# zfwangDP/X2-GNN

Hardware: AMD Instinct MI355X
Metric: molecules/sec (fwd+bwd) on QM9 U0, batch=128, 1/2/4/8 MI355X (higher is better)
Workload: dtype fp32; 1 GPU; xgnn_poly U0 train step (config.json: L=4, D=128, H=16, sbf 7x6), S160, fwd+loss+bwd+allreduce+clip+Adam+EMA; per_gpu_batch=128, global_batch=128, line_nodes_per_gpu=21058, triplets_per_gpu=194060, parallelism=dp1, hip_graph=True

## Files before the change

### x2-gnn_amd/csrc/chain.hip

```cpp
#include <math.h>

#include <type_traits>

#include "common.hpp"

namespace x2g {
namespace {

typedef float f4 __attribute__((ext_vector_type(4)));

constexpr int kCD = 128;
constexpr int kCWaves = 8;
constexpr int kCThreads = kCWaves * 64;

struct ChainFwdArgs {
  const float* x;
  const float* res;
  float* in_t;
  int64_t tf;
  int64_t R;
  int n;
  x2g_chain_stage st[X2G_CHAIN_MAX_STAGES];
};

struct ChainBwdArgs {
  const float* dy;
  const float* dy_add;
  float* dx;
  float* dres;
  float* dz_t;
  const float* ln_y;
  float2* ln_gstats;
  int64_t tf;
  int64_t R;
  int n;
  x2g_chain_bwd_stage st[X2G_CHAIN_MAX_STAGES];
};

__device__ __forceinline__ f4 zero4() { return f4{0.f, 0.f, 0.f, 0.f}; }

__device__ __forceinline__ float sigmoid_fast(float z) {
  return __builtin_amdgcn_rcpf(1.0f + __builtin_amdgcn_exp2f(-1.4426950408889634f * z));
}
__device__ __forceinline__ float silu_fast(float z) { return z * sigmoid_fast(z); }
__device__ __forceinline__ float silu_grad_fast(float z) {
  const float s = sigmoid_fast(z);
  return s * (1.0f + z * (1.0f - s));
}

constexpr int kV2RB = 6;

__device__ __forceinline__ int ipos(int r, int c) { return r * 32 + (c ^ (r & 15)); }

typedef __amdgpu_buffer_rsrc_t rsrc_t;

__device__ __forceinline__ rsrc_t rsrc(const float* p) {
  return __builtin_amdgcn_make_buffer_rsrc(const_cast<float*>(p), static_cast<short>(0), 0x7fffffff, 0x00020000);
}

__device__ __forceinline__ f4 bload4(rsrc_t r, int voff_bytes, int soff_bytes) {
  return __builtin_bit_cast(f4, __builtin_amdgcn_raw_buffer_load_b128(r, voff_bytes, soff_bytes, 0));
}

__device__ __forceinline__ float bload1(rsrc_t r, int voff_bytes, int soff_bytes) {
  return __builtin_bit_cast(float, __builtin_amdgcn_raw_buffer_load_b32(r, voff_bytes, soff_bytes, 0));
}

template <int RB = kV2RB>
__device__ __forceinline__ void stage_rows(f4* __restrict__ img, const float* __restrict__ P,
                                           const float* __restrict__ P2, int r0, int nrows) {
  const int tid = threadIdx.x;
  f4 v[RB];
#pragma unroll
  for (int u = 0; u < RB; ++u) {
    const int q = tid + kCThreads * u, r = q >> 5, c = q & 31;
    const bool ok = r < nrows;
    const int rr = r0 + (ok ? r : 0);
    v[u] = *reinterpret_cast<const f4*>(P + rr * kCD + 4 * c) * (ok ? 1.0f : 0.0f);
    if (P2) v[u] += *reinterpret_cast<const f4*>(P2 + rr * kCD + 4 * c) * (ok ? 1.0f : 0.0f);
  }
#pragma unroll
  for (int u = 0; u < RB; ++u) {
    const int q = tid + kCThreads * u;
    img[ipos(q >> 5, q & 31)] = v[u];
  }
}

template <int RB = kV2RB>
__device__ __forceinline__ void store_img(float* __restrict__ P, const f4* __restrict__ img, int r0, int nrows) {
  const int tid = threadIdx.x;
#pragma unroll
  for (int u = 0; u < RB; ++u) {
    const int q = tid + kCThreads * u, r = q >> 5, c = q & 31;
    if (r < nrows) *reinterpret_cast<f4*>(P + (r0 + r) * kCD + 4 * c) = img[ipos(r, c)];
  }
}

template <int RB>
__device__ __forceinline__ void stage_rows_async(f4* __restrict__ img, const float* __restrict__ P, int64_t R,
                                                 int r0, bool on = true) {
  static_assert(kCWaves == 8, "the swizzle repeats every 16 rows = one instruction's step");
  const int lane = threadIdx.x & 63, w = threadIdx.x >> 6;
  const rsrc_t pr = __builtin_amdgcn_make_buffer_rsrc(const_cast<float*>(P), static_cast<short>(0),
                                                      on ? static_cast<int>(R * kCD * 4) : 0, 0x00020000);
  const int r = (64 * w + lane) >> 5, c = (lane & 31) ^ (r & 15);
  const int vo = 4 * ((r0 + r) * kCD + 4 * c);
#pragma unroll
  for (int u = 0; u < RB; ++u)
    __builtin_amdgcn_raw_ptr_buffer_load_lds(pr, (__attribute__((address_space(3))) void*)(img + 64 * (8 * u + w)), 16,
                                             vo, u * 16 * kCD * 4, 0, 0);
}

__device__ __forceinline__ float dpp_xor1(float v) {
  return __builtin_bit_cast(float, __builtin_amdgcn_mov_dpp(__builtin_bit_cast(int, v), 0xB1, 0xF, 0xF, false));
}
__device__ __forceinline__ float dpp_xor2(float v) {
  return __builtin_bit_cast(float, __builtin_amdgcn_mov_dpp(__builtin_bit_cast(int, v), 0x4E, 0xF, 0xF, false));
}

template <int CTL>
__device__ __forceinline__ float dpp_f(float v) {
  return __builtin_bit_cast(float, __builtin_amdgcn_mov_dpp(__builtin_bit_cast(int, v), CTL, 0xF, 0xF, false));
}
__device__ __forceinline__ float row_sum16(float v) {
  v += dpp_f<0xB1>(v);
  v += dpp_f<0x4E>(v);
  v += dpp_f<0x141>(v);
  v += dpp_f<0x140>(v);
  return v;
}
__device__ __forceinline__ f4 quad_transpose(f4 v, int j) {
  f4 b, c;
#pragma unroll
  for (int k = 0; k < 4; ++k) {
    const float t = dpp_xor1(v[k ^ 1]);
    b[k] = ((k ^ j) & 1) ? t : v[k];
  }
#pragma unroll
  for (int k = 0; k < 4; ++k) {
    const float t = dpp_xor2(b[k ^ 2]);
    c[k] = ((k ^ j) & 2) ? t : b[k];
  }
  return c;
}

template <int RB>
__device__ __forceinline__ void store_t_slice(float* __restrict__ dst, const f4 (&v)[RB], int r0, int nrows, int w,
                                              int rl, int g) {
  const int j = rl & 3, m = rl >> 2, f = 16 * w + 4 * g + j;
  const int ntile = (nrows + 15) >> 4;
  const rsrc_t dr = __builtin_amdgcn_make_buffer_rsrc(dst, static_cast<short>(0), dst ? 0x7fffffff : 0, 0x00020000);
  const int vo = 4 * ((r0 >> 4) * (16 * kCD) + f * 16 + 4 * m);
#pragma unroll
  for (int rb = 0; rb < RB; ++rb) {
    f4 t = quad_transpose(v[rb], j);
#pragma unroll
    for (int e = 0; e < 4; ++e)
      if (16 * rb + 4 * m + e >= nrows) t[e] = 0.0f;
    __builtin_amdgcn_raw_buffer_store_b128(__builtin_bit_cast(__attribute__((ext_vector_type(4))) unsigned, t), dr,
                                           rb < ntile ? vo + rb * 4 * 16 * kCD : static_cast<int>(0x80000000u), 0, 0);
  }
}

template <bool TRANS>
__device__ __forceinline__ void load_slice(const float* W, int w, int rl, int g, f4 (&A)[8]) {
  const rsrc_t r = rsrc(W);
  if (!TRANS) {
    const int vo = 4 * ((16 * w + rl) * kCD + 4 * g);
#pragma unroll
    for (int b = 0; b < 8; ++b) A[b] = bload4(r, vo, 64 * b);
  } else {
    const int vo = 4 * (4 * g * kCD + 16 * w + rl);
#pragma unroll
    for (int b = 0; b < 8; ++b)
#pragma unroll
      for (int e = 0; e < 4; ++e) A[b][e] = bload1(r, vo, 4 * (16 * b + e) * kCD);
  }
}

template <int RB, bool ZERO = true>
__device__ __forceinline__ void slice_gemm(const f4* __restrict__ img, const f4 (&A)[8], f4 (&acc)[RB], int rl,
                                           int g) {
  if (ZERO) {
#pragma unroll
    for (int rb = 0; rb < RB; ++rb) acc[rb] = zero4();
  }
  f4 bo[2][RB];
#pragma unroll
  for (int rb = 0; rb < RB; ++rb) bo[0][rb] = img[(16 * rb + rl) * 32 + (g ^ rl)];
#pragma unroll
  for (int b = 0; b < 8; ++b) {
    const int cur = b & 1;
    if (b + 1 < 8) {
#pragma unroll
      for (int rb = 0; rb < RB; ++rb) bo[cur ^ 1][rb] = img[(16 * rb + rl) * 32 + ((4 * (b + 1) + g) ^ rl)];
    }
#pragma unroll
    for (int e = 0; e < 4; ++e)
#pragma unroll
      for (int rb = 0; rb < RB; ++rb)
        acc[rb] = __builtin_amdgcn_mfma_f32_16x16x4f32(A[b][e], bo[cur][rb][e], acc[rb], 0, 0, 0);
  }
}

template <int N>
__device__ __forceinline__ void pin(f4 (&v)[N]) {
#pragma unroll
  for (int i = 0; i < N; ++i) asm volatile("" : "+v"(v[i]));
}

__device__ __forceinline__ void chunk_rows(int64_t ch, int64_t nch, int64_t nblk, int64_t R, int& r0, int& nrows) {
  const int64_t b0 = ch * nblk / nch, b1 = (ch + 1) * nblk / nch;
  const int64_t e = b1 * 16 < R ? b1 * 16 : R;
  r0 = static_cast<int>(b0 * 16);
  nrows = static_cast<int>(e - b0 * 16);
}

constexpr int kOOB = static_cast<int>(0x80000000u);


__device__ __forceinline__ rsrc_t rsrc_n(const float* p, int64_t bytes, bool on) {
  const int64_t nr = on ? (bytes < 0x7fffffff ? bytes : 0x7fffffff) : 0;
  return __builtin_amdgcn_make_buffer_rsrc(const_cast<float*>(p), static_cast<short>(0), static_cast<int>(nr),
                                           0x00020000);
}
__device__ __forceinline__ void bstore4(rsrc_t r, f4 v, int voff_bytes) {
  __builtin_amdgcn_raw_buffer_store_b128(__builtin_bit_cast(__attribute__((ext_vector_type(4))) unsigned, v), r,
                                         voff_bytes, 0, 0);
}

template <int RB0, int RB1, int N>
__device__ __forceinline__ void half_gemm(const f4* __restrict__ img, const f4 (&A)[8], f4 (&acc)[N], int rl,
                                          int g) {
#pragma unroll
  for (int rb = RB0; rb < RB1; ++rb) acc[rb] = zero4();
#pragma unroll
  for (int b = 0; b < 8; ++b) {
    f4 bo[RB1 - RB0];
#pragma unroll
    for (int rb = RB0; rb < RB1; ++rb) bo[rb - RB0] = img[(16 * rb + rl) * 32 + ((4 * b + g) ^ rl)];
#pragma unroll
    for (int e = 0; e < 4; ++e)
#pragma unroll
      for (int rb = RB0; rb < RB1; ++rb)
        acc[rb] = __builtin_amdgcn_mfma_f32_16x16x4f32(A[b][e], bo[rb - RB0][e], acc[rb], 0, 0, 0);
  }
}

template <int RB0, int RB1, int N, bool TC = true>
__device__ __forceinline__ void half_epi(f4 (&acc)[N], const f4 (&held)[N], f4 bias, float silu_m, float res_m,
                                         rsrc_t zr, rsrc_t tr, f4* __restrict__ out, int r0, int nrows, int w,
                                         int rl, int g) {
  const int j = rl & 3, m = rl >> 2, f = 16 * w + 4 * g + j;
  const int ntile = (nrows + 15) >> 4;
#pragma unroll
  for (int rb = RB0; rb < RB1; ++rb) {
    const int r = 16 * rb + rl;
    const f4 z = acc[rb] + bias;
    if constexpr (TC) bstore4(zr, z, r < nrows ? 4 * ((r0 + r) * kCD + 16 * w + 4 * g) : kOOB);
    f4 y;
#pragma unroll
    for (int e = 0; e < 4; ++e) {
      const float sv = silu_fast(z[e]);
      y[e] = silu_m * sv + (1.0f - silu_m) * z[e] + res_m * held[rb][e];
    }
    out[ipos(r, 4 * w + g)] = y;
    acc[rb] = y;
    if constexpr (TC) {
      f4 t = quad_transpose(y, j);
#pragma unroll
      for (int e = 0; e < 4; ++e) t[e] = 16 * rb + 4 * m + e < nrows ? t[e] : 0.0f;
      bstore4(tr, t, rb < ntile ? 4 * static_cast<int>((static_cast<int64_t>(r0 >> 4) + rb) * (16 * kCD) + f * 16 + 4 * m)
                                : kOOB);
    }
  }
}

template <int BPT = 2>
__device__ __forceinline__ void interleave_epi_sched() {
#pragma unroll
  for (int b = 0; b < 8; ++b) {
    __builtin_amdgcn_sched_group_barrier(0x100, BPT, 0);
#pragma unroll
    for (int k = 0; k < 4 * BPT; ++k) {
      __builtin_amdgcn_sched_group_barrier(0x008, 1, 0);
      __builtin_amdgcn_sched_group_barrier(0x006, 3, 0);
      __builtin_amdgcn_sched_group_barrier(0x400, 1, 0);
      __builtin_amdgcn_sched_group_barrier(0x200, 1, 0);
      __builtin_amdgcn_sched_group_barrier(0x040, 1, 0);
    }
  }
}

template <int T, int BPT = 2>
__device__ __forceinline__ void frag_load(const f4* __restrict__ img, int b, int rl, int g, f4 (&bo)[BPT]) {
#pragma unroll
  for (int j = 0; j < BPT; ++j) bo[j] = img[(16 * (BPT * T + j) + rl) * 32 + ((4 * b + g) ^ rl)];
}

template <int T, int BPT, int N>
__device__ __forceinline__ void third_gemm(const f4* __restrict__ img, const f4 (&A)[8], f4 (&acc)[N],
                                           f4 (&bo)[2][BPT], int rl, int g) {
#pragma unroll
  for (int j = 0; j < BPT; ++j) acc[BPT * T + j] = zero4();
#pragma unroll
  for (int b = 0; b < 8; ++b) {
    const int cur = b & 1;
    if (b + 1 < 8)
      frag_load<T, BPT>(img, b + 1, rl, g, bo[cur ^ 1]);
    else if (T < 2)
      frag_load<(T < 2 ? T + 1 : T), BPT>(img, 0, rl, g, bo[cur ^ 1]);
#pragma unroll
    for (int e = 0; e < 4; ++e)
#pragma unroll
      for (int j = 0; j < BPT; ++j)
        acc[BPT * T + j] = __builtin_amdgcn_mfma_f32_16x16x4f32(A[b][e], bo[cur][j][e], acc[BPT * T + j], 0, 0, 0);
  }
}

template <int BPT = 2>
__device__ __forceinline__ void pipe_sched() {
#pragma unroll
  for (int b = 0; b < 8; ++b) {
    __builtin_amdgcn_sched_group_barrier(0x100, BPT, 0);
    __builtin_amdgcn_sched_group_barrier(0x008, 4 * BPT, 0);
  }
}

template <int RB, bool TC = true>
__device__ __forceinline__ void fwd4_stage(const ChainFwdArgs& a, int s, const f4* __restrict__ in,
                                           f4* __restrict__ out, const f4* __restrict__ rimg, f4 (&A)[8],
                                           f4 (&held)[RB], int r0, int nrows,
                                           int w, int rl, int g) {
  constexpr int BPT = RB / 3;
  const int n = a.n;
  const x2g_chain_stage& S = a.st[s];
  const int fl = S.flags;
  f4 An[8];
  load_slice<false>(a.st[s + 1 < n ? s + 1 : 0].w, w, rl, g, An);
  const f4 bias = bload4(rsrc(S.b ? S.b : S.w), 4 * (16 * w + 4 * g), 0) * (S.b ? 1.0f : 0.0f);
  if (fl & (X2G_CHAIN_HOLD | X2G_CHAIN_RES_EXT)) {
    const f4* src = (fl & X2G_CHAIN_HOLD) ? in : rimg;
#pragma unroll
    for (int rb = 0; rb < RB; ++rb) held[rb] = src[ipos(16 * rb + rl, 4 * w + g)];
  }
  const float silu_m = (fl & X2G_CHAIN_SILU) ? 1.0f : 0.0f;
  const float res_m = (fl & (X2G_CHAIN_RES_HELD | X2G_CHAIN_RES_EXT)) ? 1.0f : 0.0f;
  const rsrc_t zr = rsrc_n(S.z ? S.z : S.w, a.R * kCD * 4, S.z != nullptr);
  const bool t_on = a.in_t && s + 1 < n;
  const rsrc_t tr = rsrc_n(t_on ? a.in_t + (s + 1) * a.tf : S.w, a.tf * 4, t_on);
  f4 acc[RB];
  f4 bo[2][BPT];
  frag_load<0, BPT>(in, 0, rl, g, bo[0]);
  __builtin_amdgcn_sched_barrier(0);
  third_gemm<0, BPT>(in, A, acc, bo, rl, g);
  pipe_sched<BPT>();
  __builtin_amdgcn_sched_barrier(0);
  third_gemm<1, BPT>(in, A, acc, bo, rl, g);
  half_epi<0, BPT, RB, TC>(acc, held, bias, silu_m, res_m, zr, tr, out, r0, nrows, w, rl, g);
  interleave_epi_sched<BPT>();
  __builtin_amdgcn_sched_barrier(0);
  third_gemm<2, BPT>(in, A, acc, bo, rl, g);
  half_epi<BPT, 2 * BPT, RB, TC>(acc, held, bias, silu_m, res_m, zr, tr, out, r0, nrows, w, rl, g);
  interleave_epi_sched<BPT>();
  __builtin_amdgcn_sched_barrier(0);
  half_epi<2 * BPT, 3 * BPT, RB, TC>(acc, held, bias, silu_m, res_m, zr, tr, out, r0, nrows, w, rl, g);
  pin(An);
  __syncthreads();
  if (S.y) store_img<RB>(S.y, out, r0, nrows);
#pragma unroll
  for (int b = 0; b < 8; ++b) A[b] = An[b];
}

struct ChainLn {
  const float2* stats;
  const int32_t* ptr;
  float* out;
  float* mean;
  float* rstd;
  int64_t G;
  float eps;
};

__device__ __forceinline__ float wave_sum(float v) {
#pragma unroll
  for (int off = 32; off > 0; off >>= 1) v += __shfl_xor(v, off, 64);
  return v;
}

constexpr int kLongMol = 512;
template <int RB = kV2RB>
__device__ __forceinline__ void stage_rows_ln(f4* __restrict__ img, const float* __restrict__ P, int64_t R,
                                              const ChainLn& ln, float2* __restrict__ lnrow,
                                              float* __restrict__ red, int r0, int nrows) {
  const int tid = threadIdx.x, lane = tid & 63, w = tid >> 6;
  stage_rows_async<RB>(img, P, R, r0);
  constexpr int kPW = 4;
  int pk[kPW];
#pragma unroll
  for (int j = 0; j < kPW; ++j) {
    const int64_t k = lane + 64 * j;
    pk[j] = ln.ptr[k <= ln.G ? k : ln.G];
  }
  float cnt = 0.f;
#pragma unroll
  for (int j = 0; j < kPW; ++j) cnt += (lane + 64 * j <= ln.G && pk[j] <= r0) ? 1.f : 0.f;
  for (int64_t k = lane + 64 * kPW; k <= ln.G; k += 64) cnt += ln.ptr[k] <= r0 ? 1.f : 0.f;
  const int64_t m0 = static_cast<int64_t>(wave64_sum(cnt)) - 1;
  auto ptr_at = [&](int64_t k) -> int {
    if (k >= 64 * kPW) return uniform(ln.ptr[k]);
    const int l = static_cast<int>(k & 63);
    switch (k >> 6) {
      case 0: return lane_bcast(pk[0], l);
      case 1: return lane_bcast(pk[1], l);
      case 2: return lane_bcast(pk[2], l);
      default: return lane_bcast(pk[3], l);
    }
  };
  constexpr int kSW = 4;
  for (int64_t m = m0 > 0 ? m0 : 0; m < ln.G; ++m) {
    const int p0 = ptr_at(m), p1 = ptr_at(m + 1);
    if (p0 >= r0 + nrows) break;
    if (p1 - p0 <= kLongMol) continue;
    const float n = static_cast<float>(p1 - p0);
    constexpr int kU = 4;
    float s = 0.f;
    for (int base = p0 + tid; base < p1; base += kU * kCThreads) {
      float v[kU];
#pragma unroll
      for (int u = 0; u < kU; ++u) {
        const int r = base + u * kCThreads;
        v[u] = r < p1 ? ln.stats[r].x : 0.f;
      }
#pragma unroll
      for (int u = 0; u < kU; ++u) s += v[u];
    }
    s = wave64_sum(s);
    if (lane == 0) red[w] = s;
    __syncthreads();
    float st = 0.f;
#pragma unroll
    for (int ww = 0; ww < kCWaves; ++ww) st += red[ww];
    const float mu = st / n;
    float q = 0.f;
    for (int base = p0 + tid; base < p1; base += kU * kCThreads) {
      float2 v[kU];
#pragma unroll
      for (int u = 0; u < kU; ++u) {
        const int r = base + u * kCThreads;
        v[u] = r < p1 ? ln.stats[r] : make_float2(mu, 0.f);
      }
#pragma unroll
      for (int u = 0; u < kU; ++u) {
        const float d = v[u].x - mu;
        q += fmaf(static_cast<float>(kCD) * d, d, v[u].y);
      }
    }
    q = wave64_sum(q);
    if (lane == 0) red[kCWaves + w] = q;
    __syncthreads();
    float qt = 0.f;
#pragma unroll
    for (int ww = 0; ww < kCWaves; ++ww) qt += red[kCWaves + ww];
    const float denom = sqrtf(qt / (n * static_cast<float>(kCD)) + ln.eps);
    const int lo = p0 > r0 ? p0 : r0, hi = p1 < r0 + nrows ? p1 : r0 + nrows;
    for (int r = lo + tid; r < hi; r += kCThreads) lnrow[r - r0] = make_float2(mu, denom);
    if (tid == 0 && p0 >= r0) {
      if (ln.mean) ln.mean[m] = mu;
      if (ln.rstd) ln.rstd[m] = 1.0f / denom;
    }
    __syncthreads();
  }
  for (int64_t m = (m0 > 0 ? m0 : 0) + w; m < ln.G; m += kCWaves) {
    const int p0 = ptr_at(m), p1 = ptr_at(m + 1);
    if (p0 >= r0 + nrows) break;
    if (p1 <= p0 || p1 - p0 > kLongMol) continue;
    const float n = static_cast<float>(p1 - p0);
    float2 sv[kSW];
#pragma unroll
    for (int j = 0; j < kSW; ++j) {
      const int r = p0 + lane + 64 * j;
      sv[j] = ln.stats[r < p1 ? r : p0];
    }
    float s = 0.f;
#pragma unroll
    for (int j = 0; j < kSW; ++j) s += p0 + lane + 64 * j < p1 ? sv[j].x : 0.f;
    for (int r = p0 + lane + 64 * kSW; r < p1; r += 64) s += ln.stats[r].x;
    const float mu = wave64_sum(s) / n;
    float q = 0.f;
#pragma unroll
    for (int j = 0; j < kSW; ++j) {
      const float d = sv[j].x - mu;
      q += p0 + lane + 64 * j < p1 ? fmaf(static_cast<float>(kCD) * d, d, sv[j].y) : 0.f;
    }
    for (int r = p0 + lane + 64 * kSW; r < p1; r += 64) {
      const float2 st = ln.stats[r];
      const float d = st.x - mu;
      q += fmaf(static_cast<float>(kCD) * d, d, st.y);
    }
    const float denom = sqrtf(wave64_sum(q) / (n * static_cast<float>(kCD)) + ln.eps);
    const int lo = p0 > r0 ? p0 : r0, hi = p1 < r0 + nrows ? p1 : r0 + nrows;
    for (int r = lo + lane; r < hi; r += 64) lnrow[r - r0] = make_float2(mu, denom);
    if (lane == 0 && p0 >= r0) {
      if (ln.mean) ln.mean[m] = mu;
      if (ln.rstd) ln.rstd[m] = 1.0f / denom;
    }
  }
  asm volatile("s_waitcnt vmcnt(0)" ::: "memory");
  __syncthreads();
#pragma unroll
  for (int u = 0; u < RB; ++u) {
    const int q = tid + kCThreads * u, r = q >> 5, c = q & 31;
    const bool ok = r < nrows;
    const float2 st = lnrow[ok ? r : 0];
    const f4 v = img[ipos(r, c)];
    f4 y;
#pragma unroll
    for (int e = 0; e < 4; ++e) y[e] = ok ? (v[e] - st.x) / st.y : 0.0f;
    img[ipos(r, c)] = y;
    if (ln.out && ok) *reinterpret_cast<f4*>(ln.out + (r0 + r) * kCD + 4 * c) = y;
  }
}

template <bool LN, int RB = kV2RB, bool TC = true>
__device__ __forceinline__ void chain_fwd_v4_run(const ChainFwdArgs& a, const ChainLn& ln) {
  static_assert(RB == 6 || RB == 3, "thirds of 2 or 1 row blocks");
  __shared__ f4 img0[RB * 16 * 32];
  __shared__ f4 img1[RB * 16 * 32];
  __shared__ f4 imgr[RB * 16 * 32];
  __shared__ float2 lnrow[LN ? RB * 16 : 1];
  __shared__ float lnred[LN ? 2 * kCWaves : 1];
  const int tid = threadIdx.x, lane = tid & 63, w = tid >> 6;
  const int rl = lane & 15, g = lane >> 4;
  const int64_t nblk = (a.R + 15) / 16, G = gridDim.x;
  const int64_t nch = (nblk + RB * G - 1) / (RB * G) * G;
  const int n = a.n;
  for (int64_t i = static_cast<int64_t>(blockIdx.x) * kCThreads + tid; i < static_cast<int64_t>(n) * kCD * kCD;
       i += G * kCThreads) {
    const int s = static_cast<int>(i / (kCD * kCD)), e = static_cast<int>(i % (kCD * kCD));
    if (a.st[s].wt) a.st[s].wt[e] = a.st[s].w[(e % kCD) * kCD + e / kCD];
  }
  for (int64_t ch = blockIdx.x; ch < nch; ch += G) {
    int r0, nrows;
    chunk_rows(ch, nch, nblk, a.R, r0, nrows);
    __syncthreads();
    if (LN)
      stage_rows_ln<RB>(img0, a.x, a.R, ln, lnrow, lnred, r0, nrows);
    else
      stage_rows<RB>(img0, a.x, nullptr, r0, nrows);
    if (a.res) stage_rows<RB>(imgr, a.res, nullptr, r0, nrows);
    f4 A[8], held[RB];
    load_slice<false>(a.st[0].w, w, rl, g, A);
#pragma unroll
    for (int rb = 0; rb < RB; ++rb) held[rb] = zero4();
    __syncthreads();
    if (a.in_t && !(a.st[0].flags & X2G_CHAIN_IN0_ROWMAJOR)) {
      f4 xs[RB];
#pragma unroll
      for (int rb = 0; rb < RB; ++rb) xs[rb] = img0[ipos(16 * rb + rl, 4 * w + g)];
      store_t_slice(a.in_t, xs, r0, nrows, w, rl, g);
    }
    for (int s = 0; s < n; s += 2) {
      fwd4_stage<RB, TC>(a, s, img0, img1, imgr, A, held, r0, nrows, w, rl, g);
      if (s + 1 < n) fwd4_stage<RB, TC>(a, s + 1, img1, img0, imgr, A, held, r0, nrows, w, rl, g);
    }
  }
}

__global__ void __launch_bounds__(kCThreads, 1) chain_fwd_v4(const ChainFwdArgs a) { chain_fwd_v4_run<false>(a, {}); }

struct ChainFwdLnArgs {
  ChainFwdArgs a;
  ChainLn ln;
};
__global__ void __launch_bounds__(kCThreads, 1) chain_fwd_v4_ln(const ChainFwdLnArgs b) {
  chain_fwd_v4_run<true>(b.a, b.ln);
}
__global__ void __launch_bounds__(kCThreads, 1) chain_fwd_v4_ln_infer(const ChainFwdLnArgs b) {
  chain_fwd_v4_run<true, kV2RB, false>(b.a, b.ln);
}

constexpr int kChainMaxJobs = X2G_CHAIN_MAX_JOBS;
struct ChainFwdBatch {
  ChainFwdArgs a[kChainMaxJobs];
};
template <int RB>
__global__ void __launch_bounds__(kCThreads, 1) chain_fwd_v4_batch(const ChainFwdBatch b) {
  chain_fwd_v4_run<false, RB>(b.a[blockIdx.y], {});
}

template <int RB0, int RB1, int N>
__device__ __forceinline__ void bwd_elem(f4 (&gs)[N], f4 (&dh)[N], const f4 (&zc)[N], const f4 (&acc)[N],
                                         float hold_m, float held_m, float silu_m, float dres_acc_m, rsrc_t dres_r,
                                         rsrc_t dz_r, rsrc_t t_r, f4* __restrict__ out, int r0, int nrows, int w,
                                         int rl, int g) {
  const int col = 16 * w + 4 * g;
  const int j = rl & 3, m = rl >> 2, f = 16 * w + 4 * g + j;
  const int ntile = (nrows + 15) >> 4;
#pragma unroll
  for (int rb = RB0; rb < RB1; ++rb) {
    const int r = 16 * rb + rl;
    const int off = r < nrows ? 4 * ((r0 + r) * kCD + col) : kOOB;
    const f4 gv = acc[rb] + dh[rb] * hold_m;
    dh[rb] = dh[rb] * (1.0f - hold_m) + gv * held_m;
    if (dres_acc_m != 0.0f) {
      bstore4(dres_r, gv + bload4(dres_r, off, 0), off);
    } else {
      bstore4(dres_r, gv, off);
    }
    f4 dz;
#pragma unroll
    for (int e = 0; e < 4; ++e) dz[e] = gv[e] * (silu_m * silu_grad_fast(zc[rb][e]) + (1.0f - silu_m));
    bstore4(dz_r, dz, off);
    out[ipos(r, 4 * w + g)] = dz;
    gs[rb] = dz;
    f4 t = quad_transpose(dz, j);
#pragma unroll
    for (int e = 0; e < 4; ++e) t[e] = 16 * rb + 4 * m + e < nrows ? t[e] : 0.0f;
    bstore4(t_r, t, rb < ntile ? 4 * static_cast<int>((static_cast<int64_t>(r0 >> 4) + rb) * (16 * kCD) + f * 16 + 4 * m)
                               : kOOB);
  }
}

template <int RB = kV2RB>
__device__ __forceinline__ void store_img_lnstats(float* __restrict__ P, const f4* __restrict__ img,
                                                  const f4* __restrict__ yimg, float2* __restrict__ gs, int r0,
                                                  int nrows) {
  const int tid = threadIdx.x;
#pragma unroll
  for (int u = 0; u < RB; ++u) {
    const int q = tid + kCThreads * u, r = q >> 5, c = q & 31;
    const f4 g = img[ipos(r, c)], y = yimg[ipos(r, c)];
    if (r < nrows) *reinterpret_cast<f4*>(P + (r0 + r) * kCD + 4 * c) = g;
    const float s1 = half32_sum_hi((g[0] + g[1]) + (g[2] + g[3]));
    const float s2 = half32_sum_hi(fmaf(g[0], y[0], fmaf(g[1], y[1], fmaf(g[2], y[2], g[3] * y[3]))));
    if (c == 16 && r < nrows) gs[r0 + r] = make_float2(s1, s2);
  }
}

template <int RB = kV2RB>
__device__ __forceinline__ void chain_bwd_v3_run(const ChainBwdArgs& a) {
  static_assert(RB == 6 || RB == 3, "thirds of 2 or 1 row blocks");
  constexpr int BPT = RB / 3;
  __shared__ f4 img[2][RB * 16 * 32];
  __shared__ f4 yimg[RB * 16 * 32];
  const int tid = threadIdx.x, lane = tid & 63, w = tid >> 6;
  const int rl = lane & 15, g = lane >> 4;
  const int64_t nblk = (a.R + 15) / 16, G = gridDim.x;
  const int64_t nch = (nblk + RB * G - 1) / (RB * G) * G;
  const int n = a.n;
  const int col = 16 * w + 4 * g;
  for (int64_t ch = blockIdx.x; ch < nch; ch += G) {
    int r0, nrows;
    chunk_rows(ch, nch, nblk, a.R, r0, nrows);
    f4 A[8], dh[RB], zc[RB], gs[RB];
    auto load_z = [&](int s) {
      const rsrc_t zr = rsrc((a.st[s].flags & X2G_CHAIN_SILU) ? a.st[s].z : a.dy);
#pragma unroll
      for (int rb = 0; rb < RB; ++rb) {
        const int r = 16 * rb + rl;
        zc[rb] = bload4(zr, 4 * ((r0 + (r < nrows ? r : 0)) * kCD + col), 0);
      }
    };
    auto load_wslice = [&](int s, f4 (&dst)[8]) {
      if (a.st[s].wt)
        load_slice<false>(a.st[s].wt, w, rl, g, dst);
      else
        load_slice<true>(a.st[s].w, w, rl, g, dst);
    };
    auto elem_args = [&](int s, float& held_m, float& silu_m, float& dres_acc_m, rsrc_t& dres_r, rsrc_t& dz_r,
                         rsrc_t& t_r) {
      const x2g_chain_bwd_stage& S = a.st[s];
      const int fl = S.flags;
      held_m = (fl & X2G_CHAIN_RES_HELD) ? 1.0f : 0.0f;
      silu_m = (fl & X2G_CHAIN_SILU) ? 1.0f : 0.0f;
      const bool dres_on = (fl & X2G_CHAIN_RES_EXT) && a.dres;
      dres_acc_m = (fl & X2G_CHAIN_RES_ACCUM) ? 1.0f : 0.0f;
      dres_r = rsrc_n(dres_on ? a.dres : a.dy, a.R * kCD * 4, dres_on);
      dz_r = rsrc_n(S.dz ? S.dz : a.dy, a.R * kCD * 4, S.dz != nullptr);
      t_r = rsrc_n(a.dz_t ? a.dz_t + s * a.tf : a.dy, a.tf * 4, a.dz_t != nullptr);
    };
    if (a.ln_y) stage_rows_async<RB>(yimg, a.ln_y, a.R, r0);
    load_wslice(n - 1, A);
    load_z(n - 1);
    f4 acc0[RB];
    {
      const rsrc_t yr = rsrc(a.dy), ar = rsrc(a.dy_add ? a.dy_add : a.dy);
      const float am = a.dy_add ? 1.0f : 0.0f;
#pragma unroll
      for (int rb = 0; rb < RB; ++rb) {
        const int r = 16 * rb + rl;
        const int vo = 4 * ((r0 + (r < nrows ? r : 0)) * kCD + col);
        acc0[rb] = bload4(yr, vo, 0) + bload4(ar, vo, 0) * am;
        dh[rb] = zero4();
      }
    }
    int p = 0;
    __syncthreads();
    {
      float held_m, silu_m, dres_acc_m;
      rsrc_t dres_r, dz_r, t_r;
      elem_args(n - 1, held_m, silu_m, dres_acc_m, dres_r, dz_r, t_r);
      bwd_elem<0, RB>(gs, dh, zc, acc0, 0.0f, held_m, silu_m, dres_acc_m, dres_r, dz_r, t_r, img[p], r0, nrows,
                              w, rl, g);
    }
    __syncthreads();
    for (int s = n - 1; s >= 0; --s) {
      f4 An[8];
      load_wslice(s > 0 ? s - 1 : n - 1, An);
      load_z(s > 0 ? s - 1 : 0);
      const float hold_m = (a.st[s].flags & X2G_CHAIN_HOLD) ? 1.0f : 0.0f;
      const f4* in = img[p];
      f4* out = img[p ^ 1];
      f4 acc[RB];
      if (s > 0) {
        float held_m, silu_m, dres_acc_m;
        rsrc_t dres_r, dz_r, t_r;
        elem_args(s - 1, held_m, silu_m, dres_acc_m, dres_r, dz_r, t_r);
        {
          half_gemm<0, BPT>(in, A, acc, rl, g);
          __builtin_amdgcn_sched_barrier(0);
          half_gemm<BPT, 2 * BPT>(in, A, acc, rl, g);
          bwd_elem<0, BPT>(gs, dh, zc, acc, hold_m, held_m, silu_m, dres_acc_m, dres_r, dz_r, t_r, out, r0, nrows,
                            w, rl, g);
          interleave_epi_sched<BPT>();
          __builtin_amdgcn_sched_barrier(0);
          half_gemm<2 * BPT, 3 * BPT>(in, A, acc, rl, g);
          bwd_elem<BPT, 2 * BPT>(gs, dh, zc, acc, hold_m, held_m, silu_m, dres_acc_m, dres_r, dz_r, t_r, out, r0, nrows,
                            w, rl, g);
          interleave_epi_sched<BPT>();
          __builtin_amdgcn_sched_barrier(0);
          bwd_elem<2 * BPT, 3 * BPT>(gs, dh, zc, acc, hold_m, held_m, silu_m, dres_acc_m, dres_r, dz_r, t_r, out, r0, nrows,
                            w, rl, g);
        }
      } else {
        slice_gemm<RB>(in, A, acc, rl, g);
#pragma unroll
        for (int rb = 0; rb < RB; ++rb) out[ipos(16 * rb + rl, 4 * w + g)] = acc[rb] + dh[rb] * hold_m;
      }
      p ^= 1;
      pin(An);
      __syncthreads();
#pragma unroll
      for (int b = 0; b < 8; ++b) A[b] = An[b];
    }
    if (a.ln_y)
      store_img_lnstats<RB>(a.dx, img[p], yimg, a.ln_gstats, r0, nrows);
    else
      store_img<RB>(a.dx, img[p], r0, nrows);
  }
}

struct ChainBwdBatch {
  ChainBwdArgs a[kChainMaxJobs];
};
template <int RB>
__global__ void __launch_bounds__(kCThreads, 1) chain_bwd_v3_batch(const ChainBwdBatch b) {
  chain_bwd_v3_run<RB>(b.a[blockIdx.y]);
}


constexpr int kWThreads = 256;
typedef float floatx16 __attribute__((ext_vector_type(16)));

struct WgradArgs {
  x2g_wgrad_job job[X2G_CHAIN_MAX_STAGES];
  float* part_w[X2G_CHAIN_MAX_STAGES];
  float* part_b[X2G_CHAIN_MAX_STAGES];
  int64_t R;
  int chunk_rows;
};

__device__ __forceinline__ int wswz(int r, int c) { return r * 128 + 4 * ((c >> 2) ^ (r & 15)) + (c & 3); }

__device__ __forceinline__ void wtile_load(const float* __restrict__ P, int64_t r0, int64_t r1, f4 (&v)[4]) {
  const int tid = threadIdx.x, q = tid & 31;
#pragma unroll
  for (int u = 0; u < 4; ++u) {
    const int64_t r = r0 + (tid >> 5) + 8 * u;
    const bool ok = r < r1;
    const int64_t rc = ok ? r : r0;
    v[u] = *reinterpret_cast<const f4*>(P + rc * kCD + 4 * q) * (ok ? 1.0f : 0.0f);
  }
}

__device__ __forceinline__ void wtile_store(float* __restrict__ T, const f4 (&v)[4]) {
  const int tid = threadIdx.x, q = tid & 31;
#pragma unroll
  for (int u = 0; u < 4; ++u) {
    const int r = (tid >> 5) + 8 * u;
    *reinterpret_cast<f4*>(T + r * 128 + 4 * (q ^ (r & 15))) = v[u];
  }
}

__global__ void __launch_bounds__(kWThreads, 2) wgrad_batched_kernel(const WgradArgs a) {
  __shared__ __attribute__((aligned(16))) float Ds[2][32 * 128];
  __shared__ __attribute__((aligned(16))) float Xs[2][32 * 128];
  const int j = blockIdx.y;
  const x2g_wgrad_job& J = a.job[j];
  const int tid = threadIdx.x, lane = tid & 63, wave = tid >> 6, h = lane >> 5, i = lane & 31;
  const int nb = 32 * wave;
  const int64_t r0 = static_cast<int64_t>(blockIdx.x) * a.chunk_rows;
  const int64_t r1 = r0 + a.chunk_rows < a.R ? r0 + a.chunk_rows : a.R;
  floatx16 acc[4];
#pragma unroll
  for (int m = 0; m < 4; ++m)
#pragma unroll
    for (int e = 0; e < 16; ++e) acc[m][e] = 0.f;
  float bsum = 0.f;
  f4 vd[4], vx[4];
  int buf = 0;
  if (r0 < r1) {
    wtile_load(J.dy, r0, r1, vd);
    wtile_load(J.x, r0, r1, vx);
  }
  for (int64_t t = r0; t < r1; t += 32) {
    wtile_store(Ds[buf], vd);
    wtile_store(Xs[buf], vx);
    __syncthreads();
    if (t + 32 < r1) {
      wtile_load(J.dy, t + 32, r1, vd);
      wtile_load(J.x, t + 32, r1, vx);
    }
    const float* D = Ds[buf];
    const float* X = Xs[buf];
#pragma unroll
    for (int sg = 0; sg < 2; ++sg) {
#pragma unroll
      for (int s = 0; s < 8; ++s) {
        const int r = 16 * sg + s + 8 * h;
        const float av = D[wswz(r, nb + i)];
#pragma unroll
        for (int m = 0; m < 4; ++m) acc[m] = __builtin_amdgcn_mfma_f32_32x32x2f32(av, X[wswz(r, 32 * m + i)], acc[m], 0, 0, 0);
      }
    }
    if (J.db && tid < 128) {
#pragma unroll 8
      for (int rr = 0; rr < 32; ++rr) bsum += D[wswz(rr, tid)];
    }
    buf ^= 1;
  }
  float* slab = a.part_w[j] + static_cast<int64_t>(blockIdx.x) * kCD * kCD;
#pragma unroll
  for (int m = 0; m < 4; ++m)
#pragma unroll
    for (int e = 0; e < 16; ++e) slab[(nb + (e & 3) + 8 * (e >> 2) + 4 * h) * kCD + 32 * m + i] = acc[m][e];
  if (J.db && tid < 128) a.part_b[j][static_cast<int64_t>(blockIdx.x) * kCD + tid] = bsum;
}

constexpr int kWTiles = 2;

__device__ __forceinline__ int tpos(int f, int q) { return f * 4 + (q ^ (((f >> 3) & 1) * 3)); }

struct ChainWgradArgs {
  const float* in_t[X2G_CHAIN_MAX_STAGES];
  const float* dz_t[X2G_CHAIN_MAX_STAGES];
  int64_t ntiles;
  float* part_w[X2G_CHAIN_MAX_STAGES];
  float* part_b[X2G_CHAIN_MAX_STAGES];
  int has_b[X2G_CHAIN_MAX_STAGES];
  int splits;
};

template <int NB, bool SPREAD = true, int WT = kWTiles>
__device__ __forceinline__ void tiled_segment(const float* __restrict__ dz, const float* __restrict__ xin, int64_t t0,
                                              int64_t t1, bool has_b, float* __restrict__ slab,
                                              float* __restrict__ slab_b, f4 (*Ds)[WT][512],
                                              f4 (*Xs)[WT][512]) {
  const int tid = threadIdx.x, lane = tid & 63, w = tid >> 6;
  const int rl = lane & 15, g = lane >> 4;
  const int nsteps = static_cast<int>((t1 - t0 + WT - 1) / WT);
  const int P = 64 * w + lane;
  const int src_chunk = (P >> 2) * 4 + ((P & 3) ^ (((P >> 5) & 1) * 3));
  auto issue = [&](int step) {
    const int b = step % NB;
#pragma unroll
    for (int k = 0; k < WT; ++k) {
      int64_t t = t0 + static_cast<int64_t>(step) * WT + k;
      t = t < t1 ? t : t0;
      __builtin_amdgcn_global_load_lds(dz + t * 2048 + 4 * src_chunk, &Ds[b][k][64 * w], 16, 0, 0);
      __builtin_amdgcn_global_load_lds(xin + t * 2048 + 4 * src_chunk, &Xs[b][k][64 * w], 16, 0, 0);
    }
  };
  f4 acc[8];
#pragma unroll
  for (int bk = 0; bk < 8; ++bk) acc[bk] = zero4();
  float bsum = 0.f;
#pragma unroll
  for (int p = 0; p < NB - 1; ++p)
    if (p < nsteps) issue(p);
  for (int i = 0; i < nsteps; ++i) {
    const int ahead = nsteps - 1 - i < NB - 2 ? nsteps - 1 - i : NB - 2;
    if (ahead >= 2)
      asm volatile("s_waitcnt vmcnt(%0)" ::"n"(4 * WT) : "memory");
    else if (ahead == 1)
      asm volatile("s_waitcnt vmcnt(%0)" ::"n"(2 * WT) : "memory");
    else
      asm volatile("s_waitcnt vmcnt(0)" ::: "memory");
    asm volatile("s_waitcnt lgkmcnt(0)" ::: "memory");
    __builtin_amdgcn_s_barrier();
    if (i + NB - 1 < nsteps) issue(i + NB - 1);
    const int b = i % NB;
#pragma unroll
    for (int k = 0; k < WT; ++k) {
      if (t0 + static_cast<int64_t>(i) * WT + k >= t1) break;
      const f4 av = Ds[b][k][tpos(16 * w + rl, g)];
      f4 bv[8];
#pragma unroll
      for (int bk = 0; bk < 8; ++bk) bv[bk] = Xs[b][k][tpos(16 * bk + rl, g)];
#pragma unroll
      for (int e = 0; e < 4; ++e)
#pragma unroll
        for (int bk = 0; bk < 8; ++bk) acc[bk] = __builtin_amdgcn_mfma_f32_16x16x4f32(av[e], bv[bk][e], acc[bk], 0, 0, 0);
      if (SPREAD && has_b) {
        const f4 v = Ds[b][k][tpos(tid & (kCD - 1), tid >> 7)];
        bsum += (v[0] + v[1]) + (v[2] + v[3]);
      }
      if (!SPREAD && tid < 128) {
#pragma unroll
        for (int q = 0; q < 4; ++q) {
          const f4 v = Ds[b][k][tpos(tid, q)];
          bsum += (v[0] + v[1]) + (v[2] + v[3]);
        }
      }
    }
  }
#pragma unroll
  for (int bk = 0; bk < 8; ++bk)
#pragma unroll
    for (int e = 0; e < 4; ++e) slab[(16 * w + 4 * g + e) * kCD + 16 * bk + rl] = acc[bk][e];
  if (!SPREAD && has_b && tid < 128) slab_b[tid] = bsum;
  if (SPREAD && has_b) {
    __shared__ float bred[4 * kCD];
    bred[tid] = bsum;
    __syncthreads();
    if (tid < kCD) slab_b[tid] = ((bred[tid] + bred[kCD + tid]) + bred[2 * kCD + tid]) + bred[3 * kCD + tid];
  }
}

__device__ __forceinline__ int rpos(int r, int f) { return 128 * r + 4 * ((f >> 2) ^ (r & 12)) + (f & 3); }

template <bool SPREAD, int WT, bool DR, bool XR>
__device__ __forceinline__ void tiled_segment2(const float* __restrict__ dz, const float* __restrict__ xin, int64_t t0,
                                               int64_t t1, int64_t rows, bool has_b, float* __restrict__ slab,
                                               float* __restrict__ slab_b, f4 (*D0)[512], f4 (*X0)[512],
                                               f4 (*D1)[512], f4 (*X1)[512], float* __restrict__ bred) {
  const int tid = threadIdx.x, lane = tid & 63, w = tid >> 6;
  const int rl = lane & 15, g = lane >> 4;
  const int nsteps = static_cast<int>((t1 - t0 + WT - 1) / WT);
  const int P = 64 * w + lane;
  const int chunk_t = (P >> 2) * 4 + ((P & 3) ^ (((P >> 5) & 1) * 3));
  const int chunk_r = (P & ~31) | ((P & 31) ^ ((P >> 5) & 12));
  const int d_chunk = DR ? chunk_r : chunk_t, x_chunk = XR ? chunk_r : chunk_t;
  const int64_t nt = t1 - t0;
  const int nbytes = static_cast<int>(nt * 8192 < 0x7fffffff ? nt * 8192 : 0x7fffffff);
  const int64_t rend = t1 * 16 < rows ? t1 * 16 : rows;
  const int64_t rb64 = (rend - t0 * 16) * (kCD * 4);
  const int rbytes = static_cast<int>(rb64 < 0x7fffffff ? rb64 : 0x7fffffff);
  const rsrc_t dr = __builtin_amdgcn_make_buffer_rsrc(const_cast<float*>(dz + t0 * 2048), static_cast<short>(0),
                                                      DR ? rbytes : nbytes, 0x00020000);
  const rsrc_t xr = __builtin_amdgcn_make_buffer_rsrc(const_cast<float*>(xin + t0 * 2048), static_cast<short>(0),
                                                      XR ? rbytes : nbytes, 0x00020000);
  auto issue = [&](int step, f4 (*Dd)[512], f4 (*Xd)[512]) {
#pragma unroll
    for (int k = 0; k < WT; ++k) {
      int tt = step * WT + k;
      tt = tt < nt ? tt : 0;
      __builtin_amdgcn_raw_ptr_buffer_load_lds(dr, (__attribute__((address_space(3))) void*)(&Dd[k][64 * w]), 16,
                                               tt * 8192 + 16 * d_chunk, 0, 0, 0);
      __builtin_amdgcn_raw_ptr_buffer_load_lds(xr, (__attribute__((address_space(3))) void*)(&Xd[k][64 * w]), 16,
                                               tt * 8192 + 16 * x_chunk, 0, 0, 0);
    }
  };
  auto quad = [&](const f4* im, bool rowmajor, int f, int q) {
    if (!rowmajor) return im[tpos(f, q)];
    const float* fm = reinterpret_cast<const float*>(im) + rpos(4 * q, f);
    f4 v;
#pragma unroll
    for (int e = 0; e < 4; ++e) v[e] = fm[128 * e];
    return v;
  };
  int xb[4];
#pragma unroll
  for (int j = 0; j < 4; ++j) xb[j] = rpos(4 * g, 16 * j + rl);
  f4 acc[8];
#pragma unroll
  for (int bk = 0; bk < 8; ++bk) acc[bk] = zero4();
  float bsum = 0.f;
  auto body = [&](int i, f4 (*Dc)[512], f4 (*Xc)[512], f4 (*Dn)[512], f4 (*Xn)[512]) {
    asm volatile("s_waitcnt vmcnt(0)" ::: "memory");
    asm volatile("s_waitcnt lgkmcnt(0)" ::: "memory");
    __builtin_amdgcn_s_barrier();
    issue(i + 1, Dn, Xn);
#pragma unroll
    for (int k = 0; k < WT; ++k) {
      if (t0 + static_cast<int64_t>(i) * WT + k >= t1) break;
      const f4 av = quad(Dc[k], DR, 16 * w + rl, g);
      f4 bv[8];
      if (XR) {
        const float* fm = reinterpret_cast<const float*>(Xc[k]);
#pragma unroll
        for (int bk = 0; bk < 8; ++bk)
#pragma unroll
          for (int e = 0; e < 4; ++e) bv[bk][e] = fm[xb[bk & 3] + 64 * (bk >> 2) + 128 * e];
      } else {
#pragma unroll
        for (int bk = 0; bk < 8; ++bk) bv[bk] = Xc[k][tpos(16 * bk + rl, g)];
      }
#pragma unroll
      for (int e = 0; e < 4; ++e)
#pragma unroll
        for (int bk = 0; bk < 8; ++bk) acc[bk] = __builtin_amdgcn_mfma_f32_16x16x4f32(av[e], bv[bk][e], acc[bk], 0, 0, 0);
      if (SPREAD && has_b) {
        const f4 v = quad(Dc[k], DR, tid & (kCD - 1), tid >> 7);
        bsum += (v[0] + v[1]) + (v[2] + v[3]);
      }
      if (!SPREAD && tid < 128) {
#pragma unroll
        for (int q = 0; q < 4; ++q) {
          const f4 v = quad(Dc[k], DR, tid, q);
          bsum += (v[0] + v[1]) + (v[2] + v[3]);
        }
      }
    }
  };
  if (nsteps > 0) issue(0, D0, X0);
  for (int i = 0; i < nsteps; i += 2) {
    body(i, D0, X0, D1, X1);
    if (i + 1 >= nsteps) break;
    body(i + 1, D1, X1, D0, X0);
  }
  asm volatile("s_waitcnt vmcnt(0)" ::: "memory");
#pragma unroll
  for (int bk = 0; bk < 8; ++bk)
#pragma unroll
    for (int e = 0; e < 4; ++e) slab[(16 * w + 4 * g + e) * kCD + 16 * bk + rl] = acc[bk][e];
  if (!SPREAD && has_b && tid < 128) slab_b[tid] = bsum;
  if (SPREAD && has_b) {
    bred[tid] = bsum;
    __syncthreads();
    if (tid < kCD) slab_b[tid] = ((bred[tid] + bred[kCD + tid]) + bred[2 * kCD + tid]) + bred[3 * kCD + tid];
  }
}

__global__ void __launch_bounds__(kCThreads, 1) chain_wgrad_kernel(const ChainWgradArgs a) {
  __shared__ f4 Ds[3][kWTiles][512];
  __shared__ f4 Xs[3][kWTiles][512];
  const int s = blockIdx.y, c = blockIdx.x;
  const int64_t t0 = c * a.ntiles / a.splits, t1 = (c + 1) * a.ntiles / a.splits;
  tiled_segment<3>(a.dz_t[s], a.in_t[s], t0, t1, a.has_b[s] != 0, a.part_w[s] + static_cast<int64_t>(c) * kCD * kCD,
                a.part_b[s] + static_cast<int64_t>(c) * kCD, Ds, Xs);
}

struct TiledFlatArgs {
  const float* in_t[X2G_TILED_MAX_JOBS];
  const float* dz_t[X2G_TILED_MAX_JOBS];
  float* slab_w[X2G_TILED_MAX_JOBS];
  float* slab_b[X2G_TILED_MAX_JOBS];
  int wg_lo[X2G_TILED_MAX_JOBS];
  int has_b[X2G_TILED_MAX_JOBS];
  int layout[X2G_TILED_MAX_JOBS];
  int rows[X2G_TILED_MAX_JOBS];
  int64_t tile0[X2G_TILED_MAX_JOBS + 1];
  int64_t total;
  int njobs;
};

template <int NB, bool SPREAD = true, int WT = kWTiles, int WPC = 1>
__global__ void __launch_bounds__(kCThreads, 2 * WPC) tiled_flat_kernel(const TiledFlatArgs a) {
  static_assert(NB == 2, "the flat launch's two named buffers (tiled_segment2)");
  __shared__ f4 D0[WT][512];
  __shared__ f4 X0[WT][512];
  __shared__ f4 D1[WT][512];
  __shared__ f4 X1[WT][512];
  __shared__ float bred[4 * kCD];
  const int64_t G = gridDim.x, i = blockIdx.x;
  const int64_t lo = i * a.total / G, hi = (i + 1) * a.total / G;
  int j0 = 0;
  while (j0 < a.njobs && a.tile0[j0 + 1] <= lo) ++j0;
  for (int j = j0; j < a.njobs && a.tile0[j] < hi; ++j) {
    const int64_t s0 = lo > a.tile0[j] ? lo : a.tile0[j];
    const int64_t s1 = hi < a.tile0[j + 1] ? hi : a.tile0[j + 1];
    if (s0 >= s1) continue;
    __syncthreads();
    const int64_t k = i - a.wg_lo[j];
    auto seg = [&](auto dr, auto xr) {
      tiled_segment2<SPREAD, WT, decltype(dr)::value, decltype(xr)::value>(
          a.dz_t[j], a.in_t[j], s0 - a.tile0[j], s1 - a.tile0[j], a.rows[j], a.has_b[j] != 0,
          a.slab_w[j] + k * kCD * kCD, a.slab_b[j] + k * kCD, D0, X0, D1, X1, bred);
    };
    using T_ = std::false_type;
    using R_ = std::true_type;
    switch (a.layout[j]) {
      case 0: seg(T_{}, T_{}); break;
      case X2G_TILED_DY_ROWMAJOR: seg(R_{}, T_{}); break;
      case X2G_TILED_X_ROWMAJOR: seg(T_{}, R_{}); break;
      default: seg(R_{}, R_{}); break;
    }
  }
}

inline int chain_wgrad_splits_of(int64_t ntiles, int stages) {
  int64_t per = 256 / stages;
  const int64_t cap = (ntiles + 3) / 4;
  if (per > cap) per = cap;
  return static_cast<int>(per < 1 ? 1 : per);
}

constexpr int kRbfMax = 8;
constexpr int kGateRB = 3;

struct ProjFwdArgs {
  const float* x;
  const float* rbf;
  const float* wr;
  int RR;
  x2g_proj p[4];
  float* x_t;
  float* xs_t;
  int64_t R;
};

template <int RB>
__device__ __forceinline__ void load_rows_slice(const float* P, int r0, int nrows, int w, int rl, int g,
                                                f4 (&v)[RB]) {
  const rsrc_t pr = rsrc(P);
#pragma unroll
  for (int rb = 0; rb < RB; ++rb) {
    const int r = 16 * rb + rl;
    const bool ok = r < nrows;
    v[rb] = bload4(pr, 4 * ((r0 + (ok ? r : 0)) * kCD + 16 * w + 4 * g), 0) * (ok ? 1.0f : 0.0f);
  }
}

template <int NJ, int RB = kV2RB, int NT = kCThreads>
__device__ __forceinline__ void stage_rbf(float* __restrict__ srbf, const float* __restrict__ rbf, int RR, int r0,
                                          int nrows) {
  for (int i = threadIdx.x; i < RB * 16 * NJ; i += NT) {
    const int r = i / NJ, j = i % NJ;
    srbf[i] = (r < nrows && j < RR) ? rbf[static_cast<int64_t>(r0 + r) * RR + j] : 0.0f;
  }
}

template <int NJ>
__device__ __forceinline__ f4 gate_filter(const float* __restrict__ srbf, const float* __restrict__ swr, int r, int c0) {
  f4 f;
#pragma unroll
  for (int e = 0; e < 4; ++e) {
    float acc = 0.0f;
#pragma unroll
    for (int j = 0; j < NJ; ++j) acc = fmaf(swr[(c0 + e) * NJ + j], srbf[r * NJ + j], acc);
    f[e] = acc;
  }
  return f;
}

template <int NJ>
__global__ void __launch_bounds__(kCThreads, 2) conv_proj_fwd_kernel(const ProjFwdArgs a) {
  constexpr int RB = kV2RB;
  __shared__ f4 img[2][RB * 16 * 32];
  __shared__ float srbf[RB * 16 * NJ];
  __shared__ float swr[kCD * NJ];
  const int tid = threadIdx.x, lane = tid & 63, w = tid >> 6;
  const int rl = lane & 15, g = lane >> 4;
  const int64_t nblk = (a.R + 15) / 16, G = gridDim.x;
  const int64_t nch = (nblk + RB * G - 1) / (RB * G) * G;
  for (int i = tid; i < kCD * NJ; i += kCThreads) {
    const int c = i / NJ, j = i % NJ;
    swr[i] = j < a.RR ? a.wr[c * a.RR + j] : 0.0f;
  }
  for (int64_t i = static_cast<int64_t>(blockIdx.x) * kCThreads + tid; i < 4 * kCD * kCD; i += G * kCThreads) {
    const int p = static_cast<int>(i / (kCD * kCD)), e = static_cast<int>(i % (kCD * kCD));
    if (a.p[p].wt) a.p[p].wt[e] = a.p[p].w[(e % kCD) * kCD + e / kCD];
  }
  for (int64_t ch = blockIdx.x; ch < nch; ch += G) {
    int r0, nrows;
    chunk_rows(ch, nch, nblk, a.R, r0, nrows);
    __syncthreads();
    stage_rows<RB>(img[0], a.x, nullptr, r0, nrows);
    stage_rbf<NJ, RB>(srbf, a.rbf, a.RR, r0, nrows);
    f4 A[8];
    load_slice<false>(a.p[0].w, w, rl, g, A);
    __syncthreads();
    {
      f4 xv[RB], xs[RB];
#pragma unroll
      for (int rb = 0; rb < RB; ++rb) {
        const int r = 16 * rb + rl;
        xv[rb] = img[0][ipos(r, 4 * w + g)];
        xs[rb] = xv[rb] * gate_filter<NJ>(srbf, swr, r, 16 * w + 4 * g);
        img[1][ipos(r, 4 * w + g)] = xs[rb];
      }
      if (a.x_t) store_t_slice(a.x_t, xv, r0, nrows, w, rl, g);
      if (a.xs_t) store_t_slice(a.xs_t, xs, r0, nrows, w, rl, g);
    }
    __syncthreads();
#pragma unroll 1
    for (int p = 0; p < 4; ++p) {
      const x2g_proj& P = a.p[p];
      f4 An[8];
      load_slice<false>(a.p[p + 1 < 4 ? p + 1 : 0].w, w, rl, g, An);
      const f4 bias = bload4(rsrc(P.b ? P.b : P.w), 4 * (16 * w + 4 * g), 0) * (P.b ? 1.0f : 0.0f);
      f4 acc[RB];
      slice_gemm(img[(p == 1 || p == 2) ? 1 : 0], A, acc, rl, g);
#pragma unroll
      for (int rb = 0; rb < RB; ++rb) {
        const int r = 16 * rb + rl;
        if (r < nrows) *reinterpret_cast<f4*>(P.out + (r0 + r) * kCD + 16 * w + 4 * g) = acc[rb] + bias;
      }
      pin(An);
#pragma unroll
      for (int b = 0; b < 8; ++b) A[b] = An[b];
    }
  }
}

struct ProjBwdGateArgs {
  x2g_proj_grad gr[4];
  const float* dx_add;
  float* dx;
  const float* x;
  const float* rbf;
  const float* wr;
  float* drbf;
  float* part_w;
  int RR;
  int drbf_acc;
  int64_t R;
};


template <int NJ, bool TW, bool TC>
__global__ void __launch_bounds__(kCThreads, 2) conv_proj_bwd_gate_kernel(const ProjBwdGateArgs a) {
  constexpr int RB = kGateRB;
  constexpr int kImg = RB * 16 * 32;
  __shared__ f4 img_k[kImg], img_v[kImg];
  __shared__ f4 img_q[kImg], img_s[kImg];
  __shared__ float srbf[RB * 16 * NJ];
  __shared__ float swr[kCD * NJ];
  __shared__ float red[kCWaves * RB * 16 * 16];
  __shared__ float sdw[kCD * NJ];
  const int tid = threadIdx.x, lane = tid & 63, w = tid >> 6;
  const int rl = lane & 15, g = lane >> 4;
  const int64_t nblk = (a.R + 15) / 16, G = gridDim.x;
  const int64_t nch = (nblk + RB * G - 1) / (RB * G) * G;
  const int nk = static_cast<int>(nch / G);
  const int c0 = 16 * w + 4 * g;
  for (int i = tid; i < kCD * NJ; i += kCThreads) {
    const int c = i / NJ, j = i % NJ;
    swr[i] = j < a.RR ? a.wr[c * a.RR + j] : 0.0f;
    sdw[i] = 0.0f;
  }
  auto load_ws = [&](int p, f4 (&dst)[8]) {
    if (TW)
      load_slice<false>(a.gr[p].wt, w, rl, g, dst);
    else
      load_slice<true>(a.gr[p].w, w, rl, g, dst);
  };
  auto t_copy = [&](int p, const f4* im, int r0, int nrows) {
    if (!TC) return;
    f4 v[RB];
#pragma unroll
    for (int rb = 0; rb < RB; ++rb) v[rb] = im[ipos(16 * rb + rl, 4 * w + g)];
    store_t_slice(a.gr[p].g_t, v, r0, nrows, w, rl, g);
  };
  auto chunk = [&](int k, int& r0, int& nrows) { chunk_rows(blockIdx.x + k * G, nch, nblk, a.R, r0, nrows); };
  const int64_t bytes = a.R * kCD * 4;
  const rsrc_t ar = rsrc_n(a.dx_add, bytes, a.dx_add != nullptr);
  const rsrc_t dr = rsrc_n(a.dx, bytes, true);
  const rsrc_t xr = rsrc_n(a.x, bytes, true);
  const rsrc_t rr = rsrc_n(a.rbf, a.R * a.RR * 4, true);
  const rsrc_t br = rsrc_n(a.drbf, a.R * a.RR * 4, a.drbf != nullptr);
  const rsrc_t bo = rsrc_n(a.drbf, a.R * a.RR * 4, a.drbf != nullptr && a.drbf_acc);
  static_assert(RB * 16 * NJ <= kCThreads && RB * 16 * kRbfMax <= kCThreads, "one srbf / drbf element per thread");
  constexpr int kWL = TW ? 8 : 32;
  constexpr int kTS = TC ? 2 * RB : 0;
  constexpr int kKVWait = kTS + RB + 2 * kWL < 63 ? kTS + RB + 2 * kWL : 63;
  constexpr int kQSWait = kTS + 2 * kWL < 63 ? kTS + 2 * kWL : 63;
  if (nk > 0) {
    int r0, nrows;
    chunk(0, r0, nrows);
    stage_rows_async<RB>(img_k, a.gr[1].g, a.R, r0);
    stage_rows_async<RB>(img_v, a.gr[2].g, a.R, r0);
  }
  f4 A[8], An[8];
  load_ws(1, A);
  load_ws(2, An);
  __syncthreads();
  float dold = 0.0f;
  int doff = kOOB;
  auto drbf_out = [&]() {
    const int i = doff == kOOB ? 0 : tid, r = i / a.RR, j = i % a.RR;
    float sum = 0.0f;
#pragma unroll
    for (int ww = 0; ww < kCWaves; ++ww) sum += red[(ww * RB * 16 + r) * 16 + j];
    __builtin_amdgcn_raw_buffer_store_b32(__builtin_bit_cast(unsigned, dold + sum), br, doff, 0, 0);
  };
  for (int k = 0; k < nk; ++k) {
    int r0, nrows;
    chunk(k, r0, nrows);
    if (k > 0)
      asm volatile("s_waitcnt vmcnt(%0)" ::"n"(kKVWait) : "memory");
    else
      asm volatile("s_waitcnt vmcnt(0)" ::: "memory");
    __syncthreads();
    drbf_out();
    stage_rows_async<RB>(img_q, a.gr[0].g, a.R, r0);
    stage_rows_async<RB>(img_s, a.gr[3].g, a.R, r0);
    asm volatile("" ::: "memory");
    f4 xv[RB];
#pragma unroll
    for (int rb = 0; rb < RB; ++rb) {
      const int r = 16 * rb + rl;
      xv[rb] = bload4(xr, 4 * ((r0 + (r < nrows ? r : 0)) * kCD + c0), 0);
    }
    float rbv;
    {
      const int r = tid / NJ, j = tid % NJ;
      rbv = bload1(rr, (tid < RB * 16 * NJ && r < nrows && j < a.RR) ? 4 * ((r0 + r) * a.RR + j) : kOOB, 0);
    }
    if (!TC) asm volatile("" ::: "memory");
    t_copy(1, img_k, r0, nrows);
    t_copy(2, img_v, r0, nrows);
    f4 acc1[RB];
    slice_gemm(img_k, A, acc1, rl, g);
    load_ws(0, A);
    slice_gemm<RB, false>(img_v, An, acc1, rl, g);
    load_ws(3, An);
    if (tid < RB * 16 * NJ) srbf[tid] = rbv;
    asm volatile("s_waitcnt vmcnt(%0)" ::"n"(kQSWait) : "memory");
    __syncthreads();
    doff = tid < nrows * a.RR ? 4 * (r0 * a.RR + tid) : kOOB;
    dold = bload1(bo, doff, 0);
    f4 xa[RB];
#pragma unroll
    for (int rb = 0; rb < RB; ++rb) {
      const int r = 16 * rb + rl;
      xa[rb] = bload4(ar, 4 * ((r0 + (r < nrows ? r : 0)) * kCD + c0), 0);
    }
    {
      const bool more = k + 1 < nk;
      int r1, n1;
      chunk(more ? k + 1 : k, r1, n1);
      stage_rows_async<RB>(img_k, a.gr[1].g, a.R, r1, more);
      stage_rows_async<RB>(img_v, a.gr[2].g, a.R, r1, more);
      asm volatile("" ::: "memory");
    }
    t_copy(0, img_q, r0, nrows);
    t_copy(3, img_s, r0, nrows);
    f4 acc[RB], d1[RB];
    slice_gemm(img_q, A, acc, rl, g);
    load_ws(1, A);
    f4 wrv;
#pragma unroll
    for (int e = 0; e < 4; ++e) wrv[e] = swr[(c0 + e) * NJ + (rl < NJ ? rl : 0)] * (rl < NJ ? 1.0f : 0.0f);
    float aw[4][NJ];
#pragma unroll
    for (int i = 0; i < 4; ++i)
#pragma unroll
      for (int j = 0; j < NJ; ++j) aw[i][j] = 0.0f;
#pragma unroll
    for (int rb = 0; rb < RB; ++rb) {
      const int r = 16 * rb + rl;
      d1[rb] = xa[rb] + acc1[rb] * gate_filter<NJ>(srbf, swr, r, c0);
      const f4 df = r < nrows ? acc1[rb] * xv[rb] : zero4();
#pragma unroll
      for (int i = 0; i < 4; ++i)
#pragma unroll
        for (int j = 0; j < NJ; ++j) aw[i][j] = fmaf(df[i], srbf[r * NJ + j], aw[i][j]);
      f4 pd = zero4();
#pragma unroll
      for (int e = 0; e < 4; ++e) pd = __builtin_amdgcn_mfma_f32_16x16x4f32(df[e], wrv[e], pd, 0, 0, 0);
#pragma unroll
      for (int i = 0; i < 4; ++i) red[(w * RB * 16 + 16 * rb + 4 * g + i) * 16 + rl] = pd[i];
    }
#pragma unroll
    for (int i = 0; i < 4; ++i)
#pragma unroll
      for (int j = 0; j < NJ; ++j) sdw[(c0 + i) * NJ + j] += row_sum16(aw[i][j]);
    slice_gemm<RB, false>(img_s, An, acc, rl, g);
    load_ws(2, An);
#pragma unroll
    for (int rb = 0; rb < RB; ++rb) {
      const int r = 16 * rb + rl;
      bstore4(dr, d1[rb] + acc[rb], r < nrows ? 4 * ((r0 + r) * kCD + c0) : kOOB);
    }
  }
  __syncthreads();
  drbf_out();
  float* slab = a.part_w + static_cast<int64_t>(blockIdx.x) * kCD * a.RR;
  for (int i = tid; i < kCD * a.RR; i += kCThreads) slab[i] = sdw[(i / a.RR) * NJ + i % a.RR];
}

inline bool al16(const void* p) { return reinterpret_cast<uintptr_t>(p) % 16 == 0; }

inline int wgrad_chunk_rows(int64_t R, int jobs) {
  const int64_t target = 512;
  const int64_t per_job = (target + jobs - 1) / jobs;
  int64_t cr = (R + per_job - 1) / per_job;
  cr = (cr + 31) / 32 * 32;
  return static_cast<int>(cr < 64 ? 64 : cr);
}

}
}

using namespace x2g;

X2G_API int64_t x2g_chain_t_floats(int64_t rows, int32_t dim) {
  return rows > 0 && dim > 0 ? (rows + 15) / 16 * 16 * dim : 0;
}

static int chain_fwd_prepare(const float* x, const float* res_ext, const x2g_chain_stage* stages, int32_t n_stages,
                             int64_t rows, int32_t dim, float* in_t, ChainFwdArgs& a, bool& empty) {
  empty = false;
  if (!stages || n_stages < 1 || n_stages > X2G_CHAIN_MAX_STAGES || rows < 0 || dim <= 0) return X2G_EINVAL;
  if (dim != kCD || rows * kCD * 4 >= (int64_t(1) << 31)) return X2G_EUNSUPPORTED;
  a = ChainFwdArgs{};
  a.x = x;
  a.res = res_ext;
  a.in_t = in_t;
  a.tf = x2g_chain_t_floats(rows, dim);
  a.R = rows;
  a.n = n_stages;
  int n_ext = 0, held = 0;
  for (int s = 0; s < n_stages; ++s) {
    const x2g_chain_stage& S = stages[s];
    if (!S.w || (s == n_stages - 1 && !S.y)) return X2G_EINVAL;
    if (S.flags & ~(X2G_CHAIN_SILU | X2G_CHAIN_HOLD | X2G_CHAIN_RES_HELD | X2G_CHAIN_RES_EXT |
                    (s == 0 ? X2G_CHAIN_IN0_ROWMAJOR : 0)))
      return X2G_EINVAL;
    if ((S.flags & X2G_CHAIN_RES_EXT) && (S.flags & (X2G_CHAIN_HOLD | X2G_CHAIN_RES_HELD))) return X2G_EINVAL;
    if (S.flags & X2G_CHAIN_RES_EXT) held = 0;
    if (S.flags & X2G_CHAIN_HOLD) held = 1;
    if ((S.flags & X2G_CHAIN_RES_HELD) && !held) return X2G_EINVAL;
    if (S.flags & X2G_CHAIN_RES_EXT) ++n_ext;
    if (!al16(S.w) || !al16(S.b) || !al16(S.z) || !al16(S.y) || !al16(S.wt)) return X2G_EUNSUPPORTED;
    a.st[s] = S;
  }
  if (n_ext > 1 || (n_ext && !res_ext)) return X2G_EINVAL;
  if (rows == 0) {
    empty = true;
    return X2G_OK;
  }
  if (!x) return X2G_EINVAL;
  if (!al16(x) || !al16(res_ext) || !al16(in_t)) return X2G_EUNSUPPORTED;
  return X2G_OK;
}

X2G_API int x2g_chain_fwd(const float* x, const float* res_ext, const x2g_chain_stage* stages, int32_t n_stages,
                          int64_t rows, int32_t dim, float* in_t, void* stream) {
  ChainFwdArgs a{};
  bool empty;
  if (int rc = chain_fwd_prepare(x, res_ext, stages, n_stages, rows, dim, in_t, a, empty)) return rc;
  if (empty) return X2G_OK;
  hipStream_t st = as_stream(stream);
  const int64_t nblk = (rows + 15) / 16;
  chain_fwd_v4<<<static_cast<unsigned>(nblk < 256 ? nblk : 256), kCThreads, 0, st>>>(a);
  return last_launch_status();
}

X2G_API int x2g_chain_fwd_ln(const float* x, const float* row_stats, const int32_t* seg_rowptr, int64_t num_segments,
                             float eps, float* x_norm, float* seg_mean, float* seg_rstd, const float* res_ext,
                             const x2g_chain_stage* stages, int32_t n_stages, int64_t rows, int32_t dim, float* in_t,
                             void* stream) {
  ChainFwdArgs a{};
  bool empty;
  if (int rc = chain_fwd_prepare(x, res_ext, stages, n_stages, rows, dim, in_t, a, empty)) return rc;
  if (num_segments < 0 || (rows > 0 && (!row_stats || !seg_rowptr || num_segments < 1))) return X2G_EINVAL;
  if (reinterpret_cast<uintptr_t>(row_stats) % 8 || !al16(x_norm)) return X2G_EUNSUPPORTED;
  if (empty) return X2G_OK;
  const ChainFwdLnArgs b{a, {reinterpret_cast<const float2*>(row_stats), seg_rowptr, x_norm, seg_mean, seg_rstd,
                             num_segments, eps}};
  const int64_t nblk = (rows + 15) / 16;
  bool infer = b.a.in_t == nullptr;
  for (int s = 0; s < b.a.n; ++s) infer = infer && b.a.st[s].z == nullptr;
  if (infer)
    chain_fwd_v4_ln_infer<<<static_cast<unsigned>(nblk < 256 ? nblk : 256), kCThreads, 0, as_stream(stream)>>>(b);
  else
    chain_fwd_v4_ln<<<static_cast<unsigned>(nblk < 256 ? nblk : 256), kCThreads, 0, as_stream(stream)>>>(b);
  return last_launch_status();
}

static int chain_bwd_prepare(const float* dy, const float* dy_add, const x2g_chain_bwd_stage* stages, int32_t n_stages,
                             int64_t rows, int32_t dim, float* dx, float* d_res_ext, float* dz_t, ChainBwdArgs& a,
                             bool& empty, bool& res_accum) {
  empty = false;
  res_accum = false;
  if (!stages || n_stages < 1 || n_stages > X2G_CHAIN_MAX_STAGES || rows < 0 || dim <= 0) return X2G_EINVAL;
  if (dim != kCD || rows * kCD * 4 >= (int64_t(1) << 31)) return X2G_EUNSUPPORTED;
  a = ChainBwdArgs{};
  a.dy = dy;
  a.dy_add = dy_add;
  a.dx = dx;
  a.dres = d_res_ext;
  a.dz_t = dz_t;
  a.tf = x2g_chain_t_floats(rows, dim);
  a.R = rows;
  a.n = n_stages;
  int n_ext = 0, held = 0;
  for (int s = 0; s < n_stages; ++s) {
    const x2g_chain_bwd_stage& S = stages[s];
    if (!S.w || ((S.flags & X2G_CHAIN_SILU) && !S.z)) return X2G_EINVAL;
    if (S.flags & ~(X2G_CHAIN_SILU | X2G_CHAIN_HOLD | X2G_CHAIN_RES_HELD | X2G_CHAIN_RES_EXT | X2G_CHAIN_RES_ACCUM))
      return X2G_EINVAL;
    if ((S.flags & X2G_CHAIN_RES_ACCUM) && !(S.flags & X2G_CHAIN_RES_EXT)) return X2G_EINVAL;
    if ((S.flags & X2G_CHAIN_RES_EXT) && (S.flags & (X2G_CHAIN_HOLD | X2G_CHAIN_RES_HELD))) return X2G_EINVAL;
    if (S.flags & X2G_CHAIN_RES_EXT) held = 0;
    if (S.flags & X2G_CHAIN_HOLD) held = 1;
    if ((S.flags & X2G_CHAIN_RES_HELD) && !held) return X2G_EINVAL;
    if (S.flags & X2G_CHAIN_RES_EXT) ++n_ext;
    if (S.flags & X2G_CHAIN_RES_ACCUM) res_accum = true;
    if (!al16(S.w) || !al16(S.wt) || !al16(S.z) || !al16(S.dz)) return X2G_EUNSUPPORTED;
    a.st[s] = S;
  }
  if (n_ext > 1) return X2G_EINVAL;
  if (rows == 0) {
    empty = true;
    return X2G_OK;
  }
  if (!dy || !dx) return X2G_EINVAL;
  if (!al16(dy) || !al16(dy_add) || !al16(dx) || !al16(d_res_ext) || !al16(dz_t)) return X2G_EUNSUPPORTED;
  return X2G_OK;
}

static int chain_bwd_launch(const ChainBwdArgs& a, int64_t rows, void* stream) {
  hipStream_t st = as_stream(stream);
  {
    const int64_t nblk = (rows + 15) / 16;
    ChainBwdBatch b{};
    b.a[0] = a;
    const dim3 grid(static_cast<unsigned>(nblk < 256 ? nblk : 256), 1);
    chain_bwd_v3_batch<kV2RB><<<grid, kCThreads, 0, st>>>(b);
  }
  return last_launch_status();
}

X2G_API int x2g_chain_bwd_ln(const float* dy, const float* dy_add, const x2g_chain_bwd_stage* stages,
                             int32_t n_stages, int64_t rows, int32_t dim, float* dx, float* d_res_ext, float* dz_t,
                             const float* x_norm, float* row_gstats, void* stream) {
  ChainBwdArgs a{};
  bool empty, res_accum;
  if (int rc = chain_bwd_prepare(dy, dy_add, stages, n_stages, rows, dim, dx, d_res_ext, dz_t, a, empty, res_accum))
    return rc;
  if (rows > 0 && (!x_norm || !row_gstats)) return X2G_EINVAL;
  if (!al16(x_norm) || reinterpret_cast<uintptr_t>(row_gstats) % 8) return X2G_EUNSUPPORTED;
  if (empty) return X2G_OK;
  a.ln_y = x_norm;
  a.ln_gstats = reinterpret_cast<float2*>(row_gstats);
  return chain_bwd_launch(a, rows, stream);
}

X2G_API int x2g_chain_bwd(const float* dy, const float* dy_add, const x2g_chain_bwd_stage* stages, int32_t n_stages,
                          int64_t rows, int32_t dim, float* dx, float* d_res_ext, float* dz_t, void* stream) {
  ChainBwdArgs a{};
  bool empty, res_accum;
  if (int rc = chain_bwd_prepare(dy, dy_add, stages, n_stages, rows, dim, dx, d_res_ext, dz_t, a, empty, res_accum))
    return rc;
  if (empty) return X2G_OK;
  return chain_bwd_launch(a, rows, stream);
}

static inline unsigned chain_batch_grid(int64_t rows, int n_jobs) {
  const int64_t nblk = (rows + 15) / 16, per = 256 / n_jobs;
  return static_cast<unsigned>(nblk < per ? nblk : (per < 1 ? 1 : per));
}

static inline bool chain_batch_rb3(int64_t rows, unsigned grid_x) {
  const int64_t nblk = (rows + 15) / 16;
  return nblk <= 3 * static_cast<int64_t>(grid_x);
}

X2G_API int x2g_chain_fwd_batch(const x2g_chain_fwd_job* jobs, int32_t n_jobs, int32_t n_stages, int64_t rows,
                                int32_t dim, void* stream) {
  if (!jobs || n_jobs < 1 || n_jobs > kChainMaxJobs) return X2G_EINVAL;
  ChainFwdBatch b{};
  bool empty = false;
  for (int j = 0; j < n_jobs; ++j) {
    const x2g_chain_fwd_job& J = jobs[j];
    if (int rc = chain_fwd_prepare(J.x, J.res_ext, J.stages, n_stages, rows, dim, J.in_t, b.a[j], empty)) return rc;
  }
  if (empty) return X2G_OK;
  const dim3 grid(chain_batch_grid(rows, n_jobs), static_cast<unsigned>(n_jobs));
  if (chain_batch_rb3(rows, grid.x))
    chain_fwd_v4_batch<3><<<grid, kCThreads, 0, as_stream(stream)>>>(b);
  else
    chain_fwd_v4_batch<kV2RB><<<grid, kCThreads, 0, as_stream(stream)>>>(b);
  return last_launch_status();
}

X2G_API int x2g_chain_bwd_batch(const x2g_chain_bwd_job* jobs, int32_t n_jobs, int32_t n_stages, int64_t rows,
                                int32_t dim, void* stream) {
  if (!jobs || n_jobs < 1 || n_jobs > kChainMaxJobs) return X2G_EINVAL;
  ChainBwdBatch b{};
  bool empty = false, res_accum;
  for (int j = 0; j < n_jobs; ++j) {
    const x2g_chain_bwd_job& J = jobs[j];
    if (int rc = chain_bwd_prepare(J.dy, J.dy_add, J.stages, n_stages, rows, dim, J.dx, J.d_res_ext, J.dz_t, b.a[j],
                                   empty, res_accum))
      return rc;
  }
  if (empty) return X2G_OK;
  const dim3 grid(chain_batch_grid(rows, n_jobs), static_cast<unsigned>(n_jobs));
  if (chain_batch_rb3(rows, grid.x))
    chain_bwd_v3_batch<3><<<grid, kCThreads, 0, as_stream(stream)>>>(b);
  else
    chain_bwd_v3_batch<kV2RB><<<grid, kCThreads, 0, as_stream(stream)>>>(b);
  return last_launch_status();
}

X2G_API int32_t x2g_wgrad_batched_splits(int64_t rows, int32_t dim, int32_t num_jobs) {
  if (rows <= 0 || dim != kCD || num_jobs < 1 || num_jobs > X2G_CHAIN_MAX_STAGES) return 0;
  const int cr = wgrad_chunk_rows(rows, num_jobs);
  return static_cast<int32_t>((rows + cr - 1) / cr);
}

X2G_API size_t x2g_wgrad_batched_workspace(int64_t rows, int32_t dim, int32_t num_jobs) {
  const int32_t splits = x2g_wgrad_batched_splits(rows, dim, num_jobs);
  return static_cast<size_t>(num_jobs > 0 ? num_jobs : 0) * splits * (kCD * kCD + kCD) * sizeof(float);
}

X2G_API int x2g_wgrad_batched(const x2g_wgrad_job* jobs, int32_t num_jobs, int64_t rows, int32_t dim, int flags,
                              void* workspace, size_t workspace_bytes, void* stream) {
  if (!jobs || num_jobs < 1 || num_jobs > X2G_CHAIN_MAX_STAGES || rows <= 0 || dim <= 0 ||
      (flags & ~(X2G_ACCUM_WGRAD | X2G_DEFER_SLAB_SUM)))
    return X2G_EINVAL;
  if (dim != kCD || rows * kCD * 4 >= (int64_t(1) << 31)) return X2G_EUNSUPPORTED;
  const size_t need = x2g_wgrad_batched_workspace(rows, dim, num_jobs);
  if (!workspace || workspace_bytes < need) return X2G_EWORKSPACE;
  WgradArgs a{};
  a.R = rows;
  a.chunk_rows = wgrad_chunk_rows(rows, num_jobs);
  const int splits = x2g_wgrad_batched_splits(rows, dim, num_jobs);
  const size_t per_job = need / num_jobs;
  x2g_slab_job sj[X2G_CHAIN_MAX_STAGES];
  for (int j = 0; j < num_jobs; ++j) {
    const x2g_wgrad_job& J = jobs[j];
    if (!J.dy || !J.x || !J.dw) return X2G_EINVAL;
    if (!al16(J.dy) || !al16(J.x)) return X2G_EUNSUPPORTED;
    a.job[j] = J;
    a.part_w[j] = reinterpret_cast<float*>(static_cast<char*>(workspace) + per_job * j);
    a.part_b[j] = a.part_w[j] + static_cast<int64_t>(splits) * kCD * kCD;
    sj[j] = x2g_slab_job{a.part_w[j], J.db ? a.part_b[j] : nullptr, J.dw, J.db, kCD * kCD, J.db ? kCD : 0, splits};
  }
  hipStream_t st = as_stream(stream);
  wgrad_batched_kernel<<<dim3(static_cast<unsigned>(splits), static_cast<unsigned>(num_jobs)), kWThreads, 0, st>>>(a);
  const int rc = last_launch_status();
  if (rc || (flags & X2G_DEFER_SLAB_SUM)) return rc;
  return x2g_slab_sum_batch(sj, num_jobs, (flags & X2G_ACCUM_WGRAD) ? 1 : 0, stream);
}

static int32_t chain_wgrad_splits(int64_t rows, int32_t dim, int32_t n_stages) {
  if (rows <= 0 || dim != kCD || n_stages < 1 || n_stages > X2G_CHAIN_MAX_STAGES) return 0;
  return chain_wgrad_splits_of((rows + 15) / 16, n_stages);
}

X2G_API size_t x2g_chain_wgrad_workspace(int64_t rows, int32_t dim, int32_t n_stages) {
  const int32_t splits = chain_wgrad_splits(rows, dim, n_stages);
  return static_cast<size_t>(splits > 0 ? n_stages : 0) * splits * (kCD * kCD + kCD) * sizeof(float);
}

X2G_API int x2g_chain_wgrad(const float* in_t, const float* dz_t, int32_t n_stages, int64_t rows, int32_t dim,
                            float* const* dw, float* const* db, int flags, void* workspace, size_t workspace_bytes,
                            void* stream) {
  if (!in_t || !dz_t || !dw || n_stages < 1 || n_stages > X2G_CHAIN_MAX_STAGES || rows <= 0 || dim <= 0 ||
      (flags & ~(X2G_ACCUM_WGRAD | X2G_DEFER_SLAB_SUM)))
    return X2G_EINVAL;
  if (dim != kCD || rows * kCD * 4 >= (int64_t(1) << 31)) return X2G_EUNSUPPORTED;
  if (!al16(in_t) || !al16(dz_t)) return X2G_EUNSUPPORTED;
  const size_t need = x2g_chain_wgrad_workspace(rows, dim, n_stages);
  if (!workspace || workspace_bytes < need) return X2G_EWORKSPACE;
  ChainWgradArgs a{};
  const int64_t tf = x2g_chain_t_floats(rows, dim);
  for (int j = 0; j < n_stages; ++j) {
    a.in_t[j] = in_t + j * tf;
    a.dz_t[j] = dz_t + j * tf;
  }
  a.ntiles = (rows + 15) / 16;
  a.splits = chain_wgrad_splits(rows, dim, n_stages);
  const size_t per = need / n_stages;
  x2g_slab_job sj[X2G_CHAIN_MAX_STAGES];
  for (int j = 0; j < n_stages; ++j) {
    if (!dw[j]) return X2G_EINVAL;
    const bool hb = db && db[j];
    a.part_w[j] = reinterpret_cast<float*>(static_cast<char*>(workspace) + per * j);
    a.part_b[j] = a.part_w[j] + static_cast<int64_t>(a.splits) * kCD * kCD;
    a.has_b[j] = hb;
    sj[j] = x2g_slab_job{a.part_w[j], hb ? a.part_b[j] : nullptr, dw[j], hb ? db[j] : nullptr, kCD * kCD,
                         hb ? kCD : 0, a.splits};
  }
  chain_wgrad_kernel<<<dim3(static_cast<unsigned>(a.splits), static_cast<unsigned>(n_stages)), kCThreads, 0,
                       as_stream(stream)>>>(a);
  const int rc = last_launch_status();
  if (rc || (flags & X2G_DEFER_SLAB_SUM)) return rc;
  return x2g_slab_sum_batch(sj, n_stages, (flags & X2G_ACCUM_WGRAD) ? 1 : 0, stream);
}

static inline unsigned v2_grid(int64_t rows) {
  const int64_t nblk = (rows + 15) / 16;
  return static_cast<unsigned>(nblk < 256 ? nblk : 256);
}

static inline unsigned proj_grid(int64_t rows) {
  const int64_t nblk = (rows + 15) / 16, cap = 256;
  return static_cast<unsigned>(nblk < cap ? nblk : cap);
}

X2G_API int x2g_conv_proj_fwd(const float* x, const float* rbf, int32_t rbf_dim, const float* w_rbf,
                              const x2g_proj* proj, int64_t rows, int32_t dim, float* x_t, float* xs_t, void* stream) {
  if (!proj || rows < 0 || dim <= 0 || rbf_dim <= 0) return X2G_EINVAL;
  if (dim != kCD || rbf_dim > kRbfMax || rows * kCD * 4 >= (int64_t(1) << 31)) return X2G_EUNSUPPORTED;
  if (rows == 0) return X2G_OK;
  if (!x || !rbf || !w_rbf) return X2G_EINVAL;
  ProjFwdArgs a{};
  a.x = x;
  a.rbf = rbf;
  a.wr = w_rbf;
  a.RR = rbf_dim;
  a.x_t = x_t;
  a.xs_t = xs_t;
  a.R = rows;
  for (int p = 0; p < 4; ++p) {
    if (!proj[p].w || !proj[p].out) return X2G_EINVAL;
    if (!al16(proj[p].w) || !al16(proj[p].b) || !al16(proj[p].out) || !al16(proj[p].wt)) return X2G_EUNSUPPORTED;
    a.p[p] = proj[p];
  }
  if (!al16(x) || !al16(x_t) || !al16(xs_t)) return X2G_EUNSUPPORTED;
  if (rbf_dim <= 6)
    conv_proj_fwd_kernel<6><<<proj_grid(rows), kCThreads, 0, as_stream(stream)>>>(a);
  else
    conv_proj_fwd_kernel<8><<<proj_grid(rows), kCThreads, 0, as_stream(stream)>>>(a);
  return last_launch_status();
}

X2G_API int32_t x2g_conv_proj_bwd_gate_splits(int64_t rows) { return rows > 0 ? static_cast<int32_t>(proj_grid(rows)) : 0; }

X2G_API size_t x2g_conv_proj_bwd_gate_workspace(int64_t rows, int32_t rbf_dim) {
  if (rows <= 0 || rbf_dim <= 0) return 0;
  return static_cast<size_t>(proj_grid(rows)) * kCD * rbf_dim * sizeof(float);
}

X2G_API int x2g_conv_proj_bwd_gate(const x2g_proj_grad* grads, int64_t rows, int32_t dim, const float* x,
                                   const float* rbf, int32_t rbf_dim, const float* w_rbf, float* dx,
                                   const float* dx_add, float* drbf, float* dw_rbf, int flags, void* ws, size_t wsb,
                                   void* stream) {
  if (!grads || rows < 0 || dim <= 0 || rbf_dim <= 0 || !dw_rbf) return X2G_EINVAL;
  if (flags & ~(X2G_ACCUM_WGRAD | X2G_DEFER_SLAB_SUM | X2G_GATE_DRBF_ACCUM)) return X2G_EINVAL;
  if (dim != kCD || rbf_dim > kRbfMax || rows * kCD * 4 >= (int64_t(1) << 31)) return X2G_EUNSUPPORTED;
  hipStream_t st = as_stream(stream);
  if (rows == 0) {
    if (flags & X2G_DEFER_SLAB_SUM) return X2G_EINVAL;
    if (flags & X2G_ACCUM_WGRAD) return X2G_OK;
    const hipError_t e = hipMemsetAsync(dw_rbf, 0, sizeof(float) * kCD * rbf_dim, st);
    return e == hipSuccess ? X2G_OK : static_cast<int>(e);
  }
  if (!dx || !x || !rbf || !w_rbf) return X2G_EINVAL;
  if (!ws || wsb < x2g_conv_proj_bwd_gate_workspace(rows, rbf_dim)) return X2G_EWORKSPACE;
  ProjBwdGateArgs a{};
  for (int p = 0; p < 4; ++p) {
    if (!grads[p].g || !grads[p].w) return X2G_EINVAL;
    if (!al16(grads[p].g) || !al16(grads[p].w) || !al16(grads[p].wt) || !al16(grads[p].g_t)) return X2G_EUNSUPPORTED;
    a.gr[p] = grads[p];
  }
  if (!al16(dx) || !al16(dx_add) || !al16(x)) return X2G_EUNSUPPORTED;
  a.dx_add = dx_add;
  a.dx = dx;
  a.x = x;
  a.rbf = rbf;
  a.wr = w_rbf;
  a.drbf = drbf;
  a.part_w = static_cast<float*>(ws);
  a.RR = rbf_dim;
  a.drbf_acc = (flags & X2G_GATE_DRBF_ACCUM) ? 1 : 0;
  a.R = rows;
  const unsigned grid = proj_grid(rows);
  const bool tw = grads[0].wt && grads[1].wt && grads[2].wt && grads[3].wt;
  const bool tc = grads[0].g_t || grads[1].g_t || grads[2].g_t || grads[3].g_t;
  auto launch = [&](auto nj, auto tw_, auto tc_) {
    conv_proj_bwd_gate_kernel<decltype(nj)::value, decltype(tw_)::value, decltype(tc_)::value>
        <<<grid, kCThreads, 0, st>>>(a);
  };
  auto pick_tc = [&](auto nj, auto tw_) {
    if (tc)
      launch(nj, tw_, std::true_type{});
    else
      launch(nj, tw_, std::false_type{});
  };
  auto pick_tw = [&](auto nj) {
    if (tw)
      pick_tc(nj, std::true_type{});
    else
      pick_tc(nj, std::false_type{});
  };
  if (rbf_dim <= 6)
    pick_tw(std::integral_constant<int, 6>{});
  else
    pick_tw(std::integral_constant<int, 8>{});
  const int rc = last_launch_status();
  if (rc || (flags & X2G_DEFER_SLAB_SUM)) return rc;
  x2g_slab_job sj{a.part_w, nullptr, dw_rbf, nullptr, static_cast<int64_t>(kCD) * rbf_dim, 0,
                  static_cast<int32_t>(grid), 0, 0};
  return x2g_slab_sum_batch(&sj, 1, (flags & X2G_ACCUM_WGRAD) ? 1 : 0, stream);
}

constexpr int kFlatWPC = 2;
static inline unsigned flat_grid(int64_t total) {
  const int64_t cap = 256 * kFlatWPC;
  return static_cast<unsigned>(total < cap ? (total < 1 ? 1 : total) : cap);
}

static inline void flat_span(int64_t t0, int64_t t1, int64_t total, int64_t G, int& lo, int& n) {
  auto owner = [&](int64_t t) {
    int64_t i = (t * G) / total;
    while (i + 1 < G && (i + 1) * total / G <= t) ++i;
    while (i > 0 && i * total / G > t) --i;
    return static_cast<int>(i);
  };
  lo = owner(t0);
  n = owner(t1 - 1) - lo + 1;
}

static inline bool flat_tiles(const int64_t* rows, int num_jobs, int64_t* tile0) {
  tile0[0] = 0;
  for (int j = 0; j < num_jobs; ++j) {
    if (rows[j] <= 0 || rows[j] * kCD * 4 >= (int64_t(1) << 31)) return false;
    tile0[j + 1] = tile0[j] + (rows[j] + 15) / 16;
  }
  return true;
}

static size_t flat_workspace(const int64_t* rows, int32_t num_jobs, int32_t dim) {
  if (!rows || dim != kCD || num_jobs < 1 || num_jobs > X2G_TILED_MAX_JOBS) return 0;
  int64_t tile0[X2G_TILED_MAX_JOBS + 1];
  if (!flat_tiles(rows, num_jobs, tile0)) return 0;
  const int64_t total = tile0[num_jobs], G = flat_grid(total);
  int64_t slabs = 0;
  for (int j = 0; j < num_jobs; ++j) {
    int lo, n;
    flat_span(tile0[j], tile0[j + 1], total, G, lo, n);
    slabs += n;
  }
  return static_cast<size_t>(slabs) * (kCD * kCD + kCD) * sizeof(float);
}

static int flat_launch(const x2g_tiled_job* jobs, const int64_t* rows, int32_t num_jobs, int32_t dim, int flags,
                       x2g_slab_job* slab_jobs, void* workspace, size_t workspace_bytes, void* stream) {
  if (!jobs || !rows || num_jobs < 1 || num_jobs > X2G_TILED_MAX_JOBS || dim <= 0 ||
      (flags & ~(X2G_ACCUM_WGRAD | X2G_DEFER_SLAB_SUM)))
    return X2G_EINVAL;
  for (int j = 0; j < num_jobs; ++j)
    if (rows[j] <= 0) return X2G_EINVAL;
  if (dim != kCD) return X2G_EUNSUPPORTED;
  if ((flags & X2G_DEFER_SLAB_SUM) && !slab_jobs) return X2G_EINVAL;
  TiledFlatArgs a{};
  if (!flat_tiles(rows, num_jobs, a.tile0)) return X2G_EUNSUPPORTED;
  const size_t need = flat_workspace(rows, num_jobs, dim);
  if (!workspace || workspace_bytes < need) return X2G_EWORKSPACE;
  a.total = a.tile0[num_jobs];
  a.njobs = num_jobs;
  const int64_t G = flat_grid(a.total);
  x2g_slab_job sj[X2G_TILED_MAX_JOBS];
  float* base = static_cast<float*>(workspace);
  for (int j = 0; j < num_jobs; ++j) {
    const x2g_tiled_job& J = jobs[j];
    if (!J.dy_t || !J.x_t || !J.dw) return X2G_EINVAL;
    if (!al16(J.dy_t) || !al16(J.x_t)) return X2G_EUNSUPPORTED;
    if (J.ld < 0 || (J.ld > 0 && (J.cols < 1 || J.cols > kCD || J.cols > J.ld))) return X2G_EINVAL;
    if (J.layout & ~(X2G_TILED_DY_ROWMAJOR | X2G_TILED_X_ROWMAJOR)) return X2G_EINVAL;
    a.layout[j] = J.layout;
    a.rows[j] = static_cast<int>(rows[j]);
    int lo, n;
    flat_span(a.tile0[j], a.tile0[j + 1], a.total, G, lo, n);
    a.in_t[j] = J.x_t;
    a.dz_t[j] = J.dy_t;
    a.wg_lo[j] = lo;
    a.has_b[j] = J.db != nullptr;
    a.slab_w[j] = base;
    a.slab_b[j] = base + static_cast<int64_t>(n) * kCD * kCD;
    base += static_cast<int64_t>(n) * (kCD * kCD + kCD);
    sj[j] = x2g_slab_job{a.slab_w[j], J.db ? a.slab_b[j] : nullptr, J.dw, J.db, kCD * kCD, J.db ? kCD : 0, n,
                         J.ld, J.cols};
  }
  tiled_flat_kernel<2, true, 2, kFlatWPC><<<static_cast<unsigned>(G), kCThreads, 0, as_stream(stream)>>>(a);
  const int rc = last_launch_status();
  if (rc) return rc;
  if (flags & X2G_DEFER_SLAB_SUM) {
    for (int j = 0; j < num_jobs; ++j) slab_jobs[j] = sj[j];
    return X2G_OK;
  }
  return x2g_slab_sum_batch(sj, num_jobs, (flags & X2G_ACCUM_WGRAD) ? 1 : 0, stream);
}

X2G_API size_t x2g_tiled_wgrad_flat_workspace(int64_t rows, int32_t dim, int32_t num_jobs) {
  if (rows <= 0 || num_jobs < 1 || num_jobs > X2G_TILED_MAX_JOBS) return 0;
  int64_t r[X2G_TILED_MAX_JOBS];
  for (int j = 0; j < num_jobs; ++j) r[j] = rows;
  return flat_workspace(r, num_jobs, dim);
}

X2G_API int x2g_tiled_wgrad_flat(const x2g_tiled_job* jobs, int32_t num_jobs, int64_t rows, int32_t dim, int flags,
                                 x2g_slab_job* slab_jobs, void* workspace, size_t workspace_bytes, void* stream) {
  if (rows <= 0 || num_jobs < 1 || num_jobs > X2G_TILED_MAX_JOBS) return X2G_EINVAL;
  int64_t r[X2G_TILED_MAX_JOBS];
  for (int j = 0; j < num_jobs; ++j) r[j] = rows;
  return flat_launch(jobs, r, num_jobs, dim, flags, slab_jobs, workspace, workspace_bytes, stream);
}

X2G_API size_t x2g_tiled_wgrad_flat_rows_workspace(const int64_t* job_rows, int32_t num_jobs, int32_t dim) {
  return flat_workspace(job_rows, num_jobs, dim);
}

X2G_API int x2g_tiled_wgrad_flat_rows(const x2g_tiled_job* jobs, const int64_t* job_rows, int32_t num_jobs,
                                      int32_t dim, int flags, x2g_slab_job* slab_jobs, void* workspace,
                                      size_t workspace_bytes, void* stream) {
  return flat_launch(jobs, job_rows, num_jobs, dim, flags, slab_jobs, workspace, workspace_bytes, stream);
}

X2G_API size_t x2g_tiled_wgrad_workspace(int64_t rows, int32_t dim, int32_t num_jobs) {
  return x2g_chain_wgrad_workspace(rows, dim, num_jobs);
}

X2G_API int x2g_tiled_wgrad(const x2g_tiled_job* jobs, int32_t num_jobs, int64_t rows, int32_t dim, int flags,
                            void* workspace, size_t workspace_bytes, void* stream) {
  if (!jobs || num_jobs < 1 || num_jobs > X2G_CHAIN_MAX_STAGES || rows <= 0 || dim <= 0 ||
      (flags & ~(X2G_ACCUM_WGRAD | X2G_DEFER_SLAB_SUM)))
    return X2G_EINVAL;
  if (dim != kCD || rows * kCD * 4 >= (int64_t(1) << 31)) return X2G_EUNSUPPORTED;
  const size_t need = x2g_tiled_wgrad_workspace(rows, dim, num_jobs);
  if (!workspace || workspace_bytes < need) return X2G_EWORKSPACE;
  ChainWgradArgs a{};
  a.ntiles = (rows + 15) / 16;
  a.splits = chain_wgrad_splits(rows, dim, num_jobs);
  const size_t per = need / num_jobs;
  x2g_slab_job sj[X2G_CHAIN_MAX_STAGES];
  for (int j = 0; j < num_jobs; ++j) {
    const x2g_tiled_job& J = jobs[j];
    if (!J.dy_t || !J.x_t || !J.dw) return X2G_EINVAL;
    if (!al16(J.dy_t) || !al16(J.x_t)) return X2G_EUNSUPPORTED;
    if (J.layout) return X2G_EUNSUPPORTED;
    a.in_t[j] = J.x_t;
    a.dz_t[j] = J.dy_t;
    a.part_w[j] = reinterpret_cast<float*>(static_cast<char*>(workspace) + per * j);
    a.part_b[j] = a.part_w[j] + static_cast<int64_t>(a.splits) * kCD * kCD;
    a.has_b[j] = J.db != nullptr;
    if (J.ld < 0 || (J.ld > 0 && (J.cols < 1 || J.cols > kCD || J.cols > J.ld))) return X2G_EINVAL;
    sj[j] = x2g_slab_job{a.part_w[j], J.db ? a.part_b[j] : nullptr, J.dw, J.db, kCD * kCD, J.db ? kCD : 0,
                         a.splits, J.ld, J.cols};
  }
  chain_wgrad_kernel<<<dim3(static_cast<unsigned>(a.splits), static_cast<unsigned>(num_jobs)), kCThreads, 0,
                       as_stream(stream)>>>(a);
  const int rc = last_launch_status();
  if (rc || (flags & X2G_DEFER_SLAB_SUM)) return rc;
  return x2g_slab_sum_batch(sj, num_jobs, (flags & X2G_ACCUM_WGRAD) ? 1 : 0, stream);
}
```

Measured before the change: 59060 molecules/s.

## Add tail-mode row partitioning with variable row-block counts to chain kernels

Adds a partitioning mode for the fused chain MLP kernels in which each workgroup takes a fixed number of full 16-row blocks (4, 5 or 6) plus a few leftover rows (up to 4). The leftover rows are computed with scalar FMA dot products and cross-lane reductions interleaved with the MFMA pipeline. Forward, LN-forward, backward and batched launchers pick this mode when the row count fits, so that the last 16-row chunk no longer lands on a few workgroups and leaves the grid unbalanced. In exchange it adds template variants, more LDS and registers, and extra scalar work per stage.

Result: slower. 57900 molecules/s (-2.0%).

```diff
diff --git a/x2-gnn_amd/csrc/chain.hip b/x2-gnn_amd/csrc/chain.hip
--- a/x2-gnn_amd/csrc/chain.hip
+++ b/x2-gnn_amd/csrc/chain.hip
@@ -216,6 +216,115 @@
   nrows = static_cast<int>(e - b0 * 16);
 }
 
+constexpr int kTMax = 4;
+
+__host__ __device__ inline bool chain_tail_mode(int64_t R, int64_t G, int RB) {
+  const int64_t nb = R / (16 * G), rem = R - 16 * nb * G;
+  return nb == RB && (rem + G - 1) / G <= kTMax;
+}
+
+template <int RB>
+__device__ __forceinline__ void chain_part(int64_t c, int64_t G, int64_t R, int& r0, int& nrows, int& t0, int& nt) {
+  if (chain_tail_mode(R, G, RB)) {
+    const int64_t base = 16 * static_cast<int64_t>(RB) * G, rem = R - base;
+    r0 = static_cast<int>(c * RB * 16);
+    nrows = RB * 16;
+    t0 = static_cast<int>(base + c * rem / G);
+    nt = static_cast<int>(base + (c + 1) * rem / G) - t0;
+    if (nt == 0) t0 = 0;
+  } else {
+    chunk_rows(c, G, (R + 15) / 16, R, r0, nrows);
+    t0 = 0;
+    nt = 0;
+  }
+}
+
+__host__ __device__ constexpr int grp_cnt(int RB, int T) {
+  return T > 2 ? 0 : RB == 3 ? 1 : RB == 6 ? 2 : RB == 5 ? (T < 2 ? 2 : 1) : (T < 1 ? 2 : 1);
+}
+__host__ __device__ constexpr int grp_start(int RB, int T) {
+  return T == 0 ? 0 : grp_start(RB, T - 1) + grp_cnt(RB, T - 1);
+}
+
+__device__ __forceinline__ void bstore1(rsrc_t r, float v, int voff_bytes) {
+  __builtin_amdgcn_raw_buffer_store_b32(__builtin_bit_cast(unsigned, v), r, voff_bytes, 0, 0);
+}
+
+template <int RB>
+__device__ __forceinline__ void stage_tail(f4* __restrict__ img, const float* __restrict__ P, int t0, int nt) {
+  const int tid = threadIdx.x;
+  if (tid < 32 * kTMax) {
+    const int r = tid >> 5, c = tid & 31;
+    f4 v = zero4();
+    if (r < nt) v = *reinterpret_cast<const f4*>(P + (t0 + r) * kCD + 4 * c);
+    img[ipos(RB * 16 + r, c)] = v;
+  }
+}
+
+template <int RB>
+__device__ __forceinline__ void stage_tail_async(f4* __restrict__ img, const float* __restrict__ P, int64_t R, int t0) {
+  static_assert(kTMax == 4, "two waves x two rows");
+  const int lane = threadIdx.x & 63, w = threadIdx.x >> 6;
+  if (w < 2) {
+    const rsrc_t pr = __builtin_amdgcn_make_buffer_rsrc(const_cast<float*>(P), static_cast<short>(0),
+                                                        static_cast<int>(R * kCD * 4), 0x00020000);
+    const int r = 2 * w + (lane >> 5), c = (lane & 31) ^ r;
+    __builtin_amdgcn_raw_ptr_buffer_load_lds(pr, (__attribute__((address_space(3))) void*)(img + RB * 16 * 32 + 64 * w),
+                                             16, 4 * ((t0 + r) * kCD + 4 * c), 0, 0, 0);
+  }
+}
+
+template <int RB>
+__device__ __forceinline__ void store_tail(float* __restrict__ P, const f4* __restrict__ img, int t0, int nt) {
+  const int tid = threadIdx.x, r = tid >> 5, c = tid & 31;
+  if (r < nt) *reinterpret_cast<f4*>(P + (t0 + r) * kCD + 4 * c) = img[ipos(RB * 16 + r, c)];
+}
+
+template <int RB>
+__device__ __forceinline__ void tail_load(const f4* __restrict__ img, int b, int g, f4 (&x)[kTMax]) {
+#pragma unroll
+  for (int t = 0; t < kTMax; ++t) x[t] = img[(RB * 16 + t) * 32 + ((4 * b + g) ^ t)];
+}
+__device__ __forceinline__ void tail_fma(const f4 (&A)[8], int b, const f4 (&x)[kTMax], float (&p)[kTMax]) {
+#pragma unroll
+  for (int t = 0; t < kTMax; ++t)
+#pragma unroll
+    for (int e = 0; e < 4; ++e) p[t] = fmaf(A[b][e], x[t][e], p[t]);
+}
+template <int RB>
+__device__ __forceinline__ void tail_dot(const f4* __restrict__ img, const f4 (&A)[8], int b, float (&p)[kTMax],
+                                         int g) {
+  f4 x[kTMax];
+  tail_load<RB>(img, b, g, x);
+  tail_fma(A, b, x, p);
+}
+
+__device__ __forceinline__ float tail_reduce(const float (&p)[kTMax], int g) {
+  float s[kTMax];
+#pragma unroll
+  for (int t = 0; t < kTMax; ++t) {
+    typedef unsigned u2 __attribute__((ext_vector_type(2)));
+    const unsigned v = __builtin_bit_cast(unsigned, p[t]);
+    const u2 r16 = __builtin_amdgcn_permlane16_swap(v, v, false, false);
+    const float a = __builtin_bit_cast(float, r16[0]) + __builtin_bit_cast(float, r16[1]);
+    const unsigned av = __builtin_bit_cast(unsigned, a);
+    const u2 r32 = __builtin_amdgcn_permlane32_swap(av, av, false, false);
+    s[t] = __builtin_bit_cast(float, r32[0]) + __builtin_bit_cast(float, r32[1]);
+  }
+  return g == 0 ? s[0] : g == 1 ? s[1] : g == 2 ? s[2] : s[3];
+}
+
+__device__ __forceinline__ int fpos(int r, int f) { return 4 * ipos(r, f >> 2) + (f & 3); }
+
+__device__ __forceinline__ void zero_t_pad(float* __restrict__ t, int64_t tf, int p0, int p1, int64_t R) {
+  const int lo = static_cast<int>(R & 15), np = (16 - lo) & 15;
+  if (!t || !np) return;
+  for (int p = p0; p < p1; ++p) {
+    float* tile = t + p * tf + (R >> 4) * (16 * kCD);
+    for (int i = threadIdx.x; i < kCD * np; i += kCThreads) tile[(i / np) * 16 + lo + i % np] = 0.0f;
+  }
+}
+
 constexpr int kOOB = static_cast<int>(0x80000000u);
 
 
@@ -236,7 +345,7 @@
   for (int rb = RB0; rb < RB1; ++rb) acc[rb] = zero4();
 #pragma unroll
   for (int b = 0; b < 8; ++b) {
-    f4 bo[RB1 - RB0];
+    f4 bo[RB1 - RB0 > 0 ? RB1 - RB0 : 1];
 #pragma unroll
     for (int rb = RB0; rb < RB1; ++rb) bo[rb - RB0] = img[(16 * rb + rl) * 32 + ((4 * b + g) ^ rl)];
 #pragma unroll
@@ -292,29 +401,40 @@
   }
 }
 
-template <int T, int BPT = 2>
-__device__ __forceinline__ void frag_load(const f4* __restrict__ img, int b, int rl, int g, f4 (&bo)[BPT]) {
-#pragma unroll
-  for (int j = 0; j < BPT; ++j) bo[j] = img[(16 * (BPT * T + j) + rl) * 32 + ((4 * b + g) ^ rl)];
-}
-
-template <int T, int BPT, int N>
-__device__ __forceinline__ void third_gemm(const f4* __restrict__ img, const f4 (&A)[8], f4 (&acc)[N],
-                                           f4 (&bo)[2][BPT], int rl, int g) {
-#pragma unroll
-  for (int j = 0; j < BPT; ++j) acc[BPT * T + j] = zero4();
+constexpr int kGrpMax = 2;
+template <int B0, int C>
+__device__ __forceinline__ void frag_load(const f4* __restrict__ img, int b, int rl, int g, f4 (&bo)[kGrpMax]) {
+#pragma unroll
+  for (int j = 0; j < C; ++j) bo[j] = img[(16 * (B0 + j) + rl) * 32 + ((4 * b + g) ^ rl)];
+}
+
+template <int RB, int T, bool TAIL = false>
+__device__ __forceinline__ void third_gemm(const f4* __restrict__ img, const f4 (&A)[8], f4 (&acc)[RB],
+                                           f4 (&bo)[2][kGrpMax], f4 (&tx)[2][kTMax], float (&tp)[kTMax], int rl,
+                                           int g) {
+  constexpr int B0 = grp_start(RB, T), C = grp_cnt(RB, T);
+#pragma unroll
+  for (int j = 0; j < C; ++j) acc[B0 + j] = zero4();
+  if constexpr (TAIL) {
+#pragma unroll
+    for (int t = 0; t < kTMax; ++t) tp[t] = 0.0f;
+  }
 #pragma unroll
   for (int b = 0; b < 8; ++b) {
     const int cur = b & 1;
     if (b + 1 < 8)
-      frag_load<T, BPT>(img, b + 1, rl, g, bo[cur ^ 1]);
+      frag_load<B0, C>(img, b + 1, rl, g, bo[cur ^ 1]);
     else if (T < 2)
-      frag_load<(T < 2 ? T + 1 : T), BPT>(img, 0, rl, g, bo[cur ^ 1]);
+      frag_load<grp_start(RB, T + 1), grp_cnt(RB, T + 1)>(img, 0, rl, g, bo[cur ^ 1]);
+    if constexpr (TAIL) {
+      if (b + 1 < 8) tail_load<RB>(img, b + 1, g, tx[cur ^ 1]);
+      tail_fma(A, b, tx[cur], tp);
+    }
 #pragma unroll
     for (int e = 0; e < 4; ++e)
 #pragma unroll
-      for (int j = 0; j < BPT; ++j)
-        acc[BPT * T + j] = __builtin_amdgcn_mfma_f32_16x16x4f32(A[b][e], bo[cur][j][e], acc[BPT * T + j], 0, 0, 0);
+      for (int j = 0; j < C; ++j)
+        acc[B0 + j] = __builtin_amdgcn_mfma_f32_16x16x4f32(A[b][e], bo[cur][j][e], acc[B0 + j], 0, 0, 0);
   }
 }
 
@@ -327,12 +447,38 @@
   }
 }
 
-template <int RB, bool TC = true>
+template <int BPT>
+__device__ __forceinline__ void pipe_tail_sched() {
+#pragma unroll
+  for (int b = 0; b < 8; ++b) {
+    __builtin_amdgcn_sched_group_barrier(0x100, BPT + kTMax, 0);
+#pragma unroll
+    for (int k = 0; k < 4 * BPT; ++k) {
+      __builtin_amdgcn_sched_group_barrier(0x008, 1, 0);
+      __builtin_amdgcn_sched_group_barrier(0x002, 4 * kTMax / (4 * BPT), 0);
+    }
+  }
+}
+
+template <int RB, bool TC>
+__device__ __forceinline__ void tail_epi(float sum, float held_t, float bias1, float silu_m, float res_m, rsrc_t zr,
+                                         rsrc_t tr, f4* __restrict__ out, int t0, int nt, int w, int rl, int g) {
+  const int f = 16 * w + rl, row = t0 + g;
+  const bool ok = g < nt;
+  const float z = sum + bias1;
+  if constexpr (TC) bstore1(zr, z, ok ? 4 * (row * kCD + f) : kOOB);
+  const float y = silu_m * silu_fast(z) + (1.0f - silu_m) * z + res_m * held_t;
+  reinterpret_cast<float*>(out)[fpos(RB * 16 + g, f)] = y;
+  if constexpr (TC) bstore1(tr, y, ok ? 4 * ((row >> 4) * (16 * kCD) + f * 16 + (row & 15)) : kOOB);
+}
+
+template <int RB, bool TC = true, bool TAIL = false>
 __device__ __forceinline__ void fwd4_stage(const ChainFwdArgs& a, int s, const f4* __restrict__ in,
                                            f4* __restrict__ out, const f4* __restrict__ rimg, f4 (&A)[8],
-                                           f4 (&held)[RB], int r0, int nrows,
+                                           f4 (&held)[RB], float& held_t, int r0, int nrows, int t0, int nt,
                                            int w, int rl, int g) {
-  constexpr int BPT = RB / 3;
+  constexpr int C0 = grp_cnt(RB, 0), C1 = grp_cnt(RB, 1), C2 = grp_cnt(RB, 2);
+  constexpr int B1 = grp_start(RB, 1), B2 = grp_start(RB, 2);
   const int n = a.n;
   const x2g_chain_stage& S = a.st[s];
   const int fl = S.flags;
@@ -343,31 +489,45 @@
     const f4* src = (fl & X2G_CHAIN_HOLD) ? in : rimg;
 #pragma unroll
     for (int rb = 0; rb < RB; ++rb) held[rb] = src[ipos(16 * rb + rl, 4 * w + g)];
+    if constexpr (TAIL) held_t = reinterpret_cast<const float*>(src)[fpos(RB * 16 + g, 16 * w + rl)];
   }
   const float silu_m = (fl & X2G_CHAIN_SILU) ? 1.0f : 0.0f;
   const float res_m = (fl & (X2G_CHAIN_RES_HELD | X2G_CHAIN_RES_EXT)) ? 1.0f : 0.0f;
   const rsrc_t zr = rsrc_n(S.z ? S.z : S.w, a.R * kCD * 4, S.z != nullptr);
   const bool t_on = a.in_t && s + 1 < n;
   const rsrc_t tr = rsrc_n(t_on ? a.in_t + (s + 1) * a.tf : S.w, a.tf * 4, t_on);
+  float bias1 = 0.0f;
+  if constexpr (TAIL) bias1 = bload1(rsrc(S.b ? S.b : S.w), 4 * (16 * w + rl), 0) * (S.b ? 1.0f : 0.0f);
   f4 acc[RB];
-  f4 bo[2][BPT];
-  frag_load<0, BPT>(in, 0, rl, g, bo[0]);
+  f4 bo[2][kGrpMax];
+  float tp[kTMax];
+  f4 tx[2][kTMax];
+  frag_load<0, C0>(in, 0, rl, g, bo[0]);
+  if constexpr (TAIL) tail_load<RB>(in, 0, g, tx[0]);
   __builtin_amdgcn_sched_barrier(0);
-  third_gemm<0, BPT>(in, A, acc, bo, rl, g);
-  pipe_sched<BPT>();
+  third_gemm<RB, 0, TAIL>(in, A, acc, bo, tx, tp, rl, g);
+  if constexpr (TAIL)
+    pipe_tail_sched<C0>();
+  else
+    pipe_sched<C0>();
   __builtin_amdgcn_sched_barrier(0);
-  third_gemm<1, BPT>(in, A, acc, bo, rl, g);
-  half_epi<0, BPT, RB, TC>(acc, held, bias, silu_m, res_m, zr, tr, out, r0, nrows, w, rl, g);
-  interleave_epi_sched<BPT>();
+  third_gemm<RB, 1>(in, A, acc, bo, tx, tp, rl, g);
+  half_epi<0, B1, RB, TC>(acc, held, bias, silu_m, res_m, zr, tr, out, r0, nrows, w, rl, g);
+  if constexpr (TAIL)
+    tail_epi<RB, TC>(tail_reduce(tp, g), held_t, bias1, silu_m, res_m, zr, tr, out, t0, nt, w, rl, g);
+  interleave_epi_sched<C1>();
   __builtin_amdgcn_sched_barrier(0);
-  third_gemm<2, BPT>(in, A, acc, bo, rl, g);
-  half_epi<BPT, 2 * BPT, RB, TC>(acc, held, bias, silu_m, res_m, zr, tr, out, r0, nrows, w, rl, g);
-  interleave_epi_sched<BPT>();
+  third_gemm<RB, 2>(in, A, acc, bo, tx, tp, rl, g);
+  half_epi<B1, B2, RB, TC>(acc, held, bias, silu_m, res_m, zr, tr, out, r0, nrows, w, rl, g);
+  interleave_epi_sched<C2>();
   __builtin_amdgcn_sched_barrier(0);
-  half_epi<2 * BPT, 3 * BPT, RB, TC>(acc, held, bias, silu_m, res_m, zr, tr, out, r0, nrows, w, rl, g);
+  half_epi<B2, B2 + C2, RB, TC>(acc, held, bias, silu_m, res_m, zr, tr, out, r0, nrows, w, rl, g);
   pin(An);
   __syncthreads();
-  if (S.y) store_img<RB>(S.y, out, r0, nrows);
+  if (S.y) {
+    store_img<RB>(S.y, out, r0, nrows);
+    if constexpr (TAIL) store_tail<RB>(S.y, out, t0, nt);
+  }
 #pragma unroll
   for (int b = 0; b < 8; ++b) A[b] = An[b];
 }
@@ -389,12 +549,14 @@
 }
 
 constexpr int kLongMol = 512;
-template <int RB = kV2RB>
+template <int RB = kV2RB, bool TAIL = false>
 __device__ __forceinline__ void stage_rows_ln(f4* __restrict__ img, const float* __restrict__ P, int64_t R,
-                                              const ChainLn& ln, float2* __restrict__ lnrow,
-                                              float* __restrict__ red, int r0, int nrows) {
-  const int tid = threadIdx.x, lane = tid & 63, w = tid >> 6;
-  stage_rows_async<RB>(img, P, R, r0);
+                                              const ChainLn& ln, float2* __restrict__ lnrow_all,
+                                              float* __restrict__ red, int r0_blk, int nrows_blk, int t0 = 0,
+                                              int nt = 0) {
+  const int tid = threadIdx.x, lane = tid & 63, w_id = tid >> 6;
+  stage_rows_async<RB>(img, P, R, r0_blk);
+  if constexpr (TAIL) stage_tail_async<RB>(img, P, R, t0);
   constexpr int kPW = 4;
   int pk[kPW];
 #pragma unroll
@@ -402,11 +564,6 @@
     const int64_t k = lane + 64 * j;
     pk[j] = ln.ptr[k <= ln.G ? k : ln.G];
   }
-  float cnt = 0.f;
-#pragma unroll
-  for (int j = 0; j < kPW; ++j) cnt += (lane + 64 * j <= ln.G && pk[j] <= r0) ? 1.f : 0.f;
-  for (int64_t k = lane + 64 * kPW; k <= ln.G; k += 64) cnt += ln.ptr[k] <= r0 ? 1.f : 0.f;
-  const int64_t m0 = static_cast<int64_t>(wave64_sum(cnt)) - 1;
   auto ptr_at = [&](int64_t k) -> int {
     if (k >= 64 * kPW) return uniform(ln.ptr[k]);
     const int l = static_cast<int>(k & 63);
@@ -418,6 +575,12 @@
     }
   };
   constexpr int kSW = 4;
+  auto range = [&](const int r0, const int nrows, float2* __restrict__ lnrow, const int w) {
+  float cnt = 0.f;
+#pragma unroll
+  for (int j = 0; j < kPW; ++j) cnt += (lane + 64 * j <= ln.G && pk[j] <= r0) ? 1.f : 0.f;
+  for (int64_t k = lane + 64 * kPW; k <= ln.G; k += 64) cnt += ln.ptr[k] <= r0 ? 1.f : 0.f;
+  const int64_t m0 = static_cast<int64_t>(wave64_sum(cnt)) - 1;
   for (int64_t m = m0 > 0 ? m0 : 0; m < ln.G; ++m) {
     const int p0 = ptr_at(m), p1 = ptr_at(m + 1);
     if (p0 >= r0 + nrows) break;
@@ -436,7 +599,7 @@
       for (int u = 0; u < kU; ++u) s += v[u];
     }
     s = wave64_sum(s);
-    if (lane == 0) red[w] = s;
+    if (lane == 0) red[w_id] = s;
     __syncthreads();
     float st = 0.f;
 #pragma unroll
@@ -457,7 +620,7 @@
       }
     }
     q = wave64_sum(q);
-    if (lane == 0) red[kCWaves + w] = q;
+    if (lane == 0) red[kCWaves + w_id] = q;
     __syncthreads();
     float qt = 0.f;
 #pragma unroll
@@ -506,34 +669,43 @@
       if (ln.rstd) ln.rstd[m] = 1.0f / denom;
     }
   }
+  };
+  if (TAIL && nt > 0) range(t0, nt, lnrow_all + RB * 16, (w_id + 4) & 7);
+  range(r0_blk, nrows_blk, lnrow_all, w_id);
   asm volatile("s_waitcnt vmcnt(0)" ::: "memory");
   __syncthreads();
+  auto norm = [&](const int r, const int c, const int grow, const bool ok) {
+    const float2 st = lnrow_all[ok ? r : 0];
+    const f4 v = img[ipos(r, c)];
+    f4 y;
+#pragma unroll
+    for (int e = 0; e < 4; ++e) y[e] = ok ? (v[e] - st.x) / st.y : 0.0f;
+    img[ipos(r, c)] = y;
+    if (ln.out && ok) *reinterpret_cast<f4*>(ln.out + grow * kCD + 4 * c) = y;
+  };
 #pragma unroll
   for (int u = 0; u < RB; ++u) {
     const int q = tid + kCThreads * u, r = q >> 5, c = q & 31;
-    const bool ok = r < nrows;
-    const float2 st = lnrow[ok ? r : 0];
-    const f4 v = img[ipos(r, c)];
-    f4 y;
-#pragma unroll
-    for (int e = 0; e < 4; ++e) y[e] = ok ? (v[e] - st.x) / st.y : 0.0f;
-    img[ipos(r, c)] = y;
-    if (ln.out && ok) *reinterpret_cast<f4*>(ln.out + (r0 + r) * kCD + 4 * c) = y;
-  }
-}
-
-template <bool LN, int RB = kV2RB, bool TC = true>
+    norm(r, c, r0_blk + r, r < nrows_blk);
+  }
+  if constexpr (TAIL) {
+    if (tid < 32 * kTMax) norm(RB * 16 + (tid >> 5), tid & 31, t0 + (tid >> 5), (tid >> 5) < nt);
+  }
+}
+
+template <bool LN, int RB = kV2RB, bool TC = true, bool TAIL = false>
 __device__ __forceinline__ void chain_fwd_v4_run(const ChainFwdArgs& a, const ChainLn& ln) {
-  static_assert(RB == 6 || RB == 3, "thirds of 2 or 1 row blocks");
-  __shared__ f4 img0[RB * 16 * 32];
-  __shared__ f4 img1[RB * 16 * 32];
-  __shared__ f4 imgr[RB * 16 * 32];
-  __shared__ float2 lnrow[LN ? RB * 16 : 1];
+  static_assert(TAIL ? (RB >= 4 && RB <= 6) : (RB == 6 || RB == 3), "row groups of 2 or 1 row blocks");
+  constexpr int IH = RB * 16 + (TAIL ? kTMax : 0);
+  __shared__ f4 img0[IH * 32];
+  __shared__ f4 img1[IH * 32];
+  __shared__ f4 imgr[IH * 32];
+  __shared__ float2 lnrow[LN ? IH : 1];
   __shared__ float lnred[LN ? 2 * kCWaves : 1];
   const int tid = threadIdx.x, lane = tid & 63, w = tid >> 6;
   const int rl = lane & 15, g = lane >> 4;
   const int64_t nblk = (a.R + 15) / 16, G = gridDim.x;
-  const int64_t nch = (nblk + RB * G - 1) / (RB * G) * G;
+  const int64_t nch = TAIL ? G : (nblk + RB * G - 1) / (RB * G) * G;
   const int n = a.n;
   for (int64_t i = static_cast<int64_t>(blockIdx.x) * kCThreads + tid; i < static_cast<int64_t>(n) * kCD * kCD;
        i += G * kCThreads) {
@@ -541,28 +713,47 @@
     if (a.st[s].wt) a.st[s].wt[e] = a.st[s].w[(e % kCD) * kCD + e / kCD];
   }
   for (int64_t ch = blockIdx.x; ch < nch; ch += G) {
-    int r0, nrows;
-    chunk_rows(ch, nch, nblk, a.R, r0, nrows);
+    int r0, nrows, t0 = 0, nt = 0;
+    if constexpr (TAIL)
+      chain_part<RB>(ch, G, a.R, r0, nrows, t0, nt);
+    else
+      chunk_rows(ch, nch, nblk, a.R, r0, nrows);
     __syncthreads();
-    if (LN)
-      stage_rows_ln<RB>(img0, a.x, a.R, ln, lnrow, lnred, r0, nrows);
-    else
+    if (LN) {
+      stage_rows_ln<RB, TAIL>(img0, a.x, a.R, ln, lnrow, lnred, r0, nrows, t0, nt);
+    } else {
       stage_rows<RB>(img0, a.x, nullptr, r0, nrows);
-    if (a.res) stage_rows<RB>(imgr, a.res, nullptr, r0, nrows);
+      if constexpr (TAIL) stage_tail<RB>(img0, a.x, t0, nt);
+    }
+    if (a.res) {
+      stage_rows<RB>(imgr, a.res, nullptr, r0, nrows);
+      if constexpr (TAIL) stage_tail<RB>(imgr, a.res, t0, nt);
+    }
     f4 A[8], held[RB];
+    float held_t = 0.0f;
     load_slice<false>(a.st[0].w, w, rl, g, A);
 #pragma unroll
     for (int rb = 0; rb < RB; ++rb) held[rb] = zero4();
     __syncthreads();
-    if (a.in_t && !(a.st[0].flags & X2G_CHAIN_IN0_ROWMAJOR)) {
+    const bool plane0 = a.in_t && !(a.st[0].flags & X2G_CHAIN_IN0_ROWMAJOR);
+    if (plane0) {
       f4 xs[RB];
 #pragma unroll
       for (int rb = 0; rb < RB; ++rb) xs[rb] = img0[ipos(16 * rb + rl, 4 * w + g)];
       store_t_slice(a.in_t, xs, r0, nrows, w, rl, g);
+      if constexpr (TAIL) {
+        const int f = 16 * w + rl, row = t0 + g;
+        if (g < nt)
+          a.in_t[(row >> 4) * (16 * kCD) + f * 16 + (row & 15)] = reinterpret_cast<const float*>(img0)[fpos(RB * 16 + g, f)];
+      }
+    }
+    if constexpr (TAIL) {
+      if (nt > 0 && t0 + nt == a.R && TC) zero_t_pad(a.in_t, a.tf, plane0 ? 0 : 1, n, a.R);
     }
     for (int s = 0; s < n; s += 2) {
-      fwd4_stage<RB, TC>(a, s, img0, img1, imgr, A, held, r0, nrows, w, rl, g);
-      if (s + 1 < n) fwd4_stage<RB, TC>(a, s + 1, img1, img0, imgr, A, held, r0, nrows, w, rl, g);
+      fwd4_stage<RB, TC, TAIL>(a, s, img0, img1, imgr, A, held, held_t, r0, nrows, t0, nt, w, rl, g);
+      if (s + 1 < n)
+        fwd4_stage<RB, TC, TAIL>(a, s + 1, img1, img0, imgr, A, held, held_t, r0, nrows, t0, nt, w, rl, g);
     }
   }
 }
@@ -587,6 +778,23 @@
 template <int RB>
 __global__ void __launch_bounds__(kCThreads, 1) chain_fwd_v4_batch(const ChainFwdBatch b) {
   chain_fwd_v4_run<false, RB>(b.a[blockIdx.y], {});
+}
+
+template <int RB>
+__global__ void __launch_bounds__(kCThreads, 1) chain_fwd_v4t(const ChainFwdArgs a) {
+  chain_fwd_v4_run<false, RB, true, true>(a, {});
+}
+template <int RB>
+__global__ void __launch_bounds__(kCThreads, 1) chain_fwd_v4t_ln(const ChainFwdLnArgs b) {
+  chain_fwd_v4_run<true, RB, true, true>(b.a, b.ln);
+}
+template <int RB>
+__global__ void __launch_bounds__(kCThreads, 1) chain_fwd_v4t_ln_infer(const ChainFwdLnArgs b) {
+  chain_fwd_v4_run<true, RB, false, true>(b.a, b.ln);
+}
+template <int RB>
+__global__ void __launch_bounds__(kCThreads, 1) chain_fwd_v4t_batch(const ChainFwdBatch b) {
+  chain_fwd_v4_run<false, RB, true, true>(b.a[blockIdx.y], {});
 }
 
 template <int RB0, int RB1, int N>
@@ -622,6 +830,25 @@
   }
 }
 
+template <int RB>
+__device__ __forceinline__ void bwd_elem_tail(float& dh_t, float zc_t, float acc_t, float hold_m, float held_m,
+                                              float silu_m, float dres_acc_m, rsrc_t dres_r, rsrc_t dz_r, rsrc_t t_r,
+                                              f4* __restrict__ out, int t0, int nt, int w, int rl, int g) {
+  const int f = 16 * w + rl, row = t0 + g;
+  const int off = g < nt ? 4 * (row * kCD + f) : kOOB;
+  const float gv = acc_t + dh_t * hold_m;
+  dh_t = dh_t * (1.0f - hold_m) + gv * held_m;
+  if (dres_acc_m != 0.0f) {
+    bstore1(dres_r, gv + bload1(dres_r, off, 0), off);
+  } else {
+    bstore1(dres_r, gv, off);
+  }
+  const float dz = gv * (silu_m * silu_grad_fast(zc_t) + (1.0f - silu_m));
+  bstore1(dz_r, dz, off);
+  reinterpret_cast<float*>(out)[fpos(RB * 16 + g, f)] = dz;
+  bstore1(t_r, dz, g < nt ? 4 * ((row >> 4) * (16 * kCD) + f * 16 + (row & 15)) : kOOB);
+}
+
 template <int RB = kV2RB>
 __device__ __forceinline__ void store_img_lnstats(float* __restrict__ P, const f4* __restrict__ img,
                                                   const f4* __restrict__ yimg, float2* __restrict__ gs, int r0,
@@ -638,22 +865,44 @@
   }
 }
 
-template <int RB = kV2RB>
+template <int RB>
+__device__ __forceinline__ void store_tail_lnstats(float* __restrict__ P, const f4* __restrict__ img,
+                                                   const f4* __restrict__ yimg, float2* __restrict__ gs, int t0,
+                                                   int nt) {
+  const int tid = threadIdx.x;
+  if (tid < 32 * kTMax) {
+    const int r = tid >> 5, c = tid & 31;
+    const f4 g = img[ipos(RB * 16 + r, c)], y = yimg[ipos(RB * 16 + r, c)];
+    if (r < nt) *reinterpret_cast<f4*>(P + (t0 + r) * kCD + 4 * c) = g;
+    const float s1 = half32_sum_hi((g[0] + g[1]) + (g[2] + g[3]));
+    const float s2 = half32_sum_hi(fmaf(g[0], y[0], fmaf(g[1], y[1], fmaf(g[2], y[2], g[3] * y[3]))));
+    if (c == 16 && r < nt) gs[t0 + r] = make_float2(s1, s2);
+  }
+}
+
+template <int RB = kV2RB, bool TAIL = false>
 __device__ __forceinline__ void chain_bwd_v3_run(const ChainBwdArgs& a) {
-  static_assert(RB == 6 || RB == 3, "thirds of 2 or 1 row blocks");
-  constexpr int BPT = RB / 3;
-  __shared__ f4 img[2][RB * 16 * 32];
-  __shared__ f4 yimg[RB * 16 * 32];
+  static_assert(TAIL ? (RB >= 4 && RB <= 6) : (RB == 6 || RB == 3), "row groups of 2 or 1 row blocks");
+  constexpr int C1 = grp_cnt(RB, 1), C2 = grp_cnt(RB, 2);
+  constexpr int B1 = grp_start(RB, 1), B2 = grp_start(RB, 2);
+  constexpr int IH = RB * 16 + (TAIL ? kTMax : 0);
+  __shared__ f4 img[2][IH * 32];
+  __shared__ f4 yimg[IH * 32];
   const int tid = threadIdx.x, lane = tid & 63, w = tid >> 6;
   const int rl = lane & 15, g = lane >> 4;
   const int64_t nblk = (a.R + 15) / 16, G = gridDim.x;
-  const int64_t nch = (nblk + RB * G - 1) / (RB * G) * G;
+  const int64_t nch = TAIL ? G : (nblk + RB * G - 1) / (RB * G) * G;
   const int n = a.n;
   const int col = 16 * w + 4 * g;
   for (int64_t ch = blockIdx.x; ch < nch; ch += G) {
-    int r0, nrows;
-    chunk_rows(ch, nch, nblk, a.R, r0, nrows);
+    int r0, nrows, t0 = 0, nt = 0;
+    if constexpr (TAIL)
+      chain_part<RB>(ch, G, a.R, r0, nrows, t0, nt);
+    else
+      chunk_rows(ch, nch, nblk, a.R, r0, nrows);
     f4 A[8], dh[RB], zc[RB], gs[RB];
+    float dh_t = 0.0f, zc_t = 0.0f;
+    const int toff = 4 * ((t0 + (g < nt ? g : 0)) * kCD + 16 * w + rl);
     auto load_z = [&](int s) {
       const rsrc_t zr = rsrc((a.st[s].flags & X2G_CHAIN_SILU) ? a.st[s].z : a.dy);
 #pragma unroll
@@ -661,6 +910,7 @@
         const int r = 16 * rb + rl;
         zc[rb] = bload4(zr, 4 * ((r0 + (r < nrows ? r : 0)) * kCD + col), 0);
       }
+      if constexpr (TAIL) zc_t = bload1(zr, toff, 0);
     };
     auto load_wslice = [&](int s, f4 (&dst)[8]) {
       if (a.st[s].wt)
@@ -680,10 +930,14 @@
       dz_r = rsrc_n(S.dz ? S.dz : a.dy, a.R * kCD * 4, S.dz != nullptr);
       t_r = rsrc_n(a.dz_t ? a.dz_t + s * a.tf : a.dy, a.tf * 4, a.dz_t != nullptr);
     };
-    if (a.ln_y) stage_rows_async<RB>(yimg, a.ln_y, a.R, r0);
+    if (a.ln_y) {
+      stage_rows_async<RB>(yimg, a.ln_y, a.R, r0);
+      if constexpr (TAIL) stage_tail_async<RB>(yimg, a.ln_y, a.R, t0);
+    }
     load_wslice(n - 1, A);
     load_z(n - 1);
     f4 acc0[RB];
+    float acc0_t = 0.0f;
     {
       const rsrc_t yr = rsrc(a.dy), ar = rsrc(a.dy_add ? a.dy_add : a.dy);
       const float am = a.dy_add ? 1.0f : 0.0f;
@@ -694,6 +948,10 @@
         acc0[rb] = bload4(yr, vo, 0) + bload4(ar, vo, 0) * am;
         dh[rb] = zero4();
       }
+      if constexpr (TAIL) acc0_t = bload1(yr, toff, 0) + bload1(ar, toff, 0) * am;
+    }
+    if constexpr (TAIL) {
+      if (nt > 0 && t0 + nt == a.R) zero_t_pad(a.dz_t, a.tf, 0, n, a.R);
     }
     int p = 0;
     __syncthreads();
@@ -703,6 +961,9 @@
       elem_args(n - 1, held_m, silu_m, dres_acc_m, dres_r, dz_r, t_r);
       bwd_elem<0, RB>(gs, dh, zc, acc0, 0.0f, held_m, silu_m, dres_acc_m, dres_r, dz_r, t_r, img[p], r0, nrows,
                               w, rl, g);
+      if constexpr (TAIL)
+        bwd_elem_tail<RB>(dh_t, zc_t, acc0_t, 0.0f, held_m, silu_m, dres_acc_m, dres_r, dz_r, t_r, img[p], t0, nt, w,
+                          rl, g);
     }
     __syncthreads();
     for (int s = n - 1; s >= 0; --s) {
@@ -718,25 +979,72 @@
         rsrc_t dres_r, dz_r, t_r;
         elem_args(s - 1, held_m, silu_m, dres_acc_m, dres_r, dz_r, t_r);
         {
-          half_gemm<0, BPT>(in, A, acc, rl, g);
+          float tp[kTMax];
+          if constexpr (TAIL) {
+#pragma unroll
+            for (int rb = 0; rb < B1; ++rb) acc[rb] = zero4();
+#pragma unroll
+            for (int t = 0; t < kTMax; ++t) tp[t] = 0.0f;
+            f4 tx[2][kTMax];
+            tail_load<RB>(in, 0, g, tx[0]);
+            __builtin_amdgcn_sched_barrier(0);
+#pragma unroll
+            for (int b = 0; b < 8; ++b) {
+              f4 bo[B1];
+#pragma unroll
+              for (int rb = 0; rb < B1; ++rb) bo[rb] = in[(16 * rb + rl) * 32 + ((4 * b + g) ^ rl)];
+              if (b + 1 < 8) tail_load<RB>(in, b + 1, g, tx[(b & 1) ^ 1]);
+              tail_fma(A, b, tx[b & 1], tp);
+#pragma unroll
+              for (int e = 0; e < 4; ++e)
+#pragma unroll
+                for (int rb = 0; rb < B1; ++rb)
+                  acc[rb] = __builtin_amdgcn_mfma_f32_16x16x4f32(A[b][e], bo[rb][e], acc[rb], 0, 0, 0);
+            }
+            pipe_tail_sched<B1>();
+          } else {
+            half_gemm<0, B1>(in, A, acc, rl, g);
+          }
           __builtin_amdgcn_sched_barrier(0);
-          half_gemm<BPT, 2 * BPT>(in, A, acc, rl, g);
-          bwd_elem<0, BPT>(gs, dh, zc, acc, hold_m, held_m, silu_m, dres_acc_m, dres_r, dz_r, t_r, out, r0, nrows,
+          float tsum = 0.0f;
+          if constexpr (TAIL) {
+            tsum = tail_reduce(tp, g);
+            __builtin_amdgcn_sched_barrier(0);
+          }
+          half_gemm<B1, B2>(in, A, acc, rl, g);
+          bwd_elem<0, B1>(gs, dh, zc, acc, hold_m, held_m, silu_m, dres_acc_m, dres_r, dz_r, t_r, out, r0, nrows,
                             w, rl, g);
-          interleave_epi_sched<BPT>();
+          if constexpr (TAIL)
+            bwd_elem_tail<RB>(dh_t, zc_t, tsum, hold_m, held_m, silu_m, dres_acc_m, dres_r, dz_r, t_r, out, t0, nt, w,
+                              rl, g);
+          interleave_epi_sched<C1>();
           __builtin_amdgcn_sched_barrier(0);
-          half_gemm<2 * BPT, 3 * BPT>(in, A, acc, rl, g);
-          bwd_elem<BPT, 2 * BPT>(gs, dh, zc, acc, hold_m, held_m, silu_m, dres_acc_m, dres_r, dz_r, t_r, out, r0, nrows,
+          half_gemm<B2, B2 + C2>(in, A, acc, rl, g);
+          bwd_elem<B1, B2>(gs, dh, zc, acc, hold_m, held_m, silu_m, dres_acc_m, dres_r, dz_r, t_r, out, r0, nrows,
                             w, rl, g);
-          interleave_epi_sched<BPT>();
+          interleave_epi_sched<C2>();
           __builtin_amdgcn_sched_barrier(0);
-          bwd_elem<2 * BPT, 3 * BPT>(gs, dh, zc, acc, hold_m, held_m, silu_m, dres_acc_m, dres_r, dz_r, t_r, out, r0, nrows,
+          bwd_elem<B2, B2 + C2>(gs, dh, zc, acc, hold_m, held_m, silu_m, dres_acc_m, dres_r, dz_r, t_r, out, r0, nrows,
                             w, rl, g);
         }
       } else {
         slice_gemm<RB>(in, A, acc, rl, g);
 #pragma unroll
         for (int rb = 0; rb < RB; ++rb) out[ipos(16 * rb + rl, 4 * w + g)] = acc[rb] + dh[rb] * hold_m;
+        if constexpr (TAIL) {
+          __builtin_amdgcn_sched_barrier(0);
+          float tp[kTMax];
+#pragma unroll
+          for (int t = 0; t < kTMax; ++t) tp[t] = 0.0f;
+#pragma unroll
+          for (int b = 0; b < 8; ++b) tail_dot<RB>(in, A, b, tp, g);
+#pragma unroll
+          for (int b = 0; b < 8; ++b) {
+            __builtin_amdgcn_sched_group_barrier(0x100, kTMax, 0);
+            __builtin_amdgcn_sched_group_barrier(0x002, 4 * kTMax, 0);
+          }
+          reinterpret_cast<float*>(out)[fpos(RB * 16 + g, 16 * w + rl)] = tail_reduce(tp, g) + dh_t * hold_m;
+        }
       }
       p ^= 1;
       pin(An);
@@ -744,10 +1052,13 @@
 #pragma unroll
       for (int b = 0; b < 8; ++b) A[b] = An[b];
     }
-    if (a.ln_y)
+    if (a.ln_y) {
       store_img_lnstats<RB>(a.dx, img[p], yimg, a.ln_gstats, r0, nrows);
-    else
+      if constexpr (TAIL) store_tail_lnstats<RB>(a.dx, img[p], yimg, a.ln_gstats, t0, nt);
+    } else {
       store_img<RB>(a.dx, img[p], r0, nrows);
+      if constexpr (TAIL) store_tail<RB>(a.dx, img[p], t0, nt);
+    }
   }
 }
 
@@ -757,6 +1068,10 @@
 template <int RB>
 __global__ void __launch_bounds__(kCThreads, 1) chain_bwd_v3_batch(const ChainBwdBatch b) {
   chain_bwd_v3_run<RB>(b.a[blockIdx.y]);
+}
+template <int RB>
+__global__ void __launch_bounds__(kCThreads, 1) chain_bwd_v3t_batch(const ChainBwdBatch b) {
+  chain_bwd_v3_run<RB, true>(b.a[blockIdx.y]);
 }
 
 
@@ -1448,6 +1763,19 @@
   return X2G_OK;
 }
 
+static int chain_plan_rb(int64_t rows, int64_t G) {
+  const int64_t nblk = (rows + 15) / 16, nb = rows / (16 * G), mb = (nblk + G - 1) / G;
+  if (nb >= 4 && nb <= 6 && chain_tail_mode(rows, G, static_cast<int>(nb))) return static_cast<int>(nb);
+  return mb == 4 || mb == 5 ? static_cast<int>(mb) : 0;
+}
+
+template <class F>
+static void chain_rb_switch(int rb, F&& f) {
+  if (rb == 4) f(std::integral_constant<int, 4>{});
+  if (rb == 5) f(std::integral_constant<int, 5>{});
+  if (rb == 6) f(std::integral_constant<int, 6>{});
+}
+
 X2G_API int x2g_chain_fwd(const float* x, const float* res_ext, const x2g_chain_stage* stages, int32_t n_stages,
                           int64_t rows, int32_t dim, float* in_t, void* stream) {
   ChainFwdArgs a{};
@@ -1456,7 +1784,11 @@
   if (empty) return X2G_OK;
   hipStream_t st = as_stream(stream);
   const int64_t nblk = (rows + 15) / 16;
-  chain_fwd_v4<<<static_cast<unsigned>(nblk < 256 ? nblk : 256), kCThreads, 0, st>>>(a);
+  const unsigned G = static_cast<unsigned>(nblk < 256 ? nblk : 256);
+  if (const int rb = chain_plan_rb(rows, G))
+    chain_rb_switch(rb, [&](auto RB) { chain_fwd_v4t<decltype(RB)::value><<<G, kCThreads, 0, st>>>(a); });
+  else
+    chain_fwd_v4<<<G, kCThreads, 0, st>>>(a);
   return last_launch_status();
 }
 
@@ -1475,10 +1807,17 @@
   const int64_t nblk = (rows + 15) / 16;
   bool infer = b.a.in_t == nullptr;
   for (int s = 0; s < b.a.n; ++s) infer = infer && b.a.st[s].z == nullptr;
-  if (infer)
-    chain_fwd_v4_ln_infer<<<static_cast<unsigned>(nblk < 256 ? nblk : 256), kCThreads, 0, as_stream(stream)>>>(b);
+  const unsigned G = static_cast<unsigned>(nblk < 256 ? nblk : 256);
+  hipStream_t st = as_stream(stream);
+  const int rb = chain_plan_rb(rows, G);
+  if (rb && infer)
+    chain_rb_switch(rb, [&](auto RB) { chain_fwd_v4t_ln_infer<decltype(RB)::value><<<G, kCThreads, 0, st>>>(b); });
+  else if (rb)
+    chain_rb_switch(rb, [&](auto RB) { chain_fwd_v4t_ln<decltype(RB)::value><<<G, kCThreads, 0, st>>>(b); });
+  else if (infer)
+    chain_fwd_v4_ln_infer<<<G, kCThreads, 0, st>>>(b);
   else
-    chain_fwd_v4_ln<<<static_cast<unsigned>(nblk < 256 ? nblk : 256), kCThreads, 0, as_stream(stream)>>>(b);
+    chain_fwd_v4_ln<<<G, kCThreads, 0, st>>>(b);
   return last_launch_status();
 }
 
@@ -1531,7 +1870,10 @@
     ChainBwdBatch b{};
     b.a[0] = a;
     const dim3 grid(static_cast<unsigned>(nblk < 256 ? nblk : 256), 1);
-    chain_bwd_v3_batch<kV2RB><<<grid, kCThreads, 0, st>>>(b);
+    if (const int rb = chain_plan_rb(rows, grid.x))
+      chain_rb_switch(rb, [&](auto RB) { chain_bwd_v3t_batch<decltype(RB)::value><<<grid, kCThreads, 0, st>>>(b); });
+    else
+      chain_bwd_v3_batch<kV2RB><<<grid, kCThreads, 0, st>>>(b);
   }
   return last_launch_status();
 }
@@ -1582,10 +1924,13 @@
   }
   if (empty) return X2G_OK;
   const dim3 grid(chain_batch_grid(rows, n_jobs), static_cast<unsigned>(n_jobs));
+  hipStream_t st = as_stream(stream);
   if (chain_batch_rb3(rows, grid.x))
-    chain_fwd_v4_batch<3><<<grid, kCThreads, 0, as_stream(stream)>>>(b);
+    chain_fwd_v4_batch<3><<<grid, kCThreads, 0, st>>>(b);
+  else if (const int rb = chain_plan_rb(rows, grid.x))
+    chain_rb_switch(rb, [&](auto RB) { chain_fwd_v4t_batch<decltype(RB)::value><<<grid, kCThreads, 0, st>>>(b); });
   else
-    chain_fwd_v4_batch<kV2RB><<<grid, kCThreads, 0, as_stream(stream)>>>(b);
+    chain_fwd_v4_batch<kV2RB><<<grid, kCThreads, 0, st>>>(b);
   return last_launch_status();
 }
 
@@ -1602,10 +1947,13 @@
   }
   if (empty) return X2G_OK;
   const dim3 grid(chain_batch_grid(rows, n_jobs), static_cast<unsigned>(n_jobs));
+  hipStream_t st = as_stream(stream);
   if (chain_batch_rb3(rows, grid.x))
-    chain_bwd_v3_batch<3><<<grid, kCThreads, 0, as_stream(stream)>>>(b);
+    chain_bwd_v3_batch<3><<<grid, kCThreads, 0, st>>>(b);
+  else if (const int rb = chain_plan_rb(rows, grid.x))
+    chain_rb_switch(rb, [&](auto RB) { chain_bwd_v3t_batch<decltype(RB)::value><<<grid, kCThreads, 0, st>>>(b); });
   else
-    chain_bwd_v3_batch<kV2RB><<<grid, kCThreads, 0, as_stream(stream)>>>(b);
+    chain_bwd_v3_batch<kV2RB><<<grid, kCThreads, 0, st>>>(b);
   return last_launch_status();
 }
 
```
